# Baverne/VAE-CYCLEGAN-Implementation

Hardware: AMD Instinct MI355X
Metric: train images/sec (256x256 VAE-CycleGAN step) (higher is better)
Workload: dtype f32; 1 GPU; cyclevaegan unpaired, 3x256x256 synthetic summer<->winter, per-GPU batch 8, latent 64 (BASELINE.json configs[3]/[4]); per_gpu_batch=8, global_batch=8, image_size=256, latent_dim=64, parallelism=dp1, init=random (reference init statistics)

## Files before the change

include/vcg.h:

```cpp
#ifndef VCG_H
#define VCG_H

#include <stddef.h>
#include <stdint.h>

#ifdef __cplusplus
extern "C" {
#endif

#define VCG_ABI_VERSION 6

void vcg_amax_hint(uint64_t x_amax, uint64_t dy_amax);
uint64_t vcg_amax_last(void);
uint64_t vcg_amax_measure(const float* t, size_t n, void* stream);
int vcg_amax_valid(uint64_t handle);

enum {
  VCG_CD_N = 0,
  VCG_CD_H = 1,
  VCG_CD_W = 2,
  VCG_CD_CIN = 3,
  VCG_CD_COUT = 4,
  VCG_CD_KH = 5,
  VCG_CD_KW = 6,
  VCG_CD_STRIDE = 7,
  VCG_CD_PAD = 8,
  VCG_CD_REFLECT = 9,
  VCG_CD_UPS = 10,
  VCG_CD_ACT = 11,
  VCG_CD_CIN_LOGICAL = 12,
  VCG_CD_COUT_LOGICAL = 13,
  VCG_CD_PACK_FLAGS = 14,
  VCG_CD_LEN = 16
};

enum { VCG_ACT_NONE = 0, VCG_ACT_RELU = 1, VCG_ACT_LEAKY02 = 2, VCG_ACT_TANH = 3, VCG_ACT_SIGMOID = 4 };

int vcg_abi_version(void);
const char* vcg_last_error(void);

int vcg_profile_enable(int on);
long vcg_profile_read(char* buf, size_t cap);

int vcg_nchw_to_nhwc(const float* src, float* dst, int N, int C, int H, int W, int P, void* stream);
int vcg_nhwc_to_nchw(const float* src, float* dst, int N, int C, int H, int W, int P, void* stream);
int vcg_fill(float* dst, float value, size_t n, void* stream);

size_t vcg_pack_weight_floats(const int32_t* cd);
int vcg_conv_reads_wf(const int32_t* cd);
int vcg_pack_weight(const float* w_oihw, float* wf, const int32_t* cd, void* stream);
size_t vcg_conv_fwd_workspace(const int32_t* cd);
int vcg_conv_fwd(const float* x, const float* wf, const float* bias, float* y,
                 const int32_t* cd, void* ws, size_t ws_bytes, void* stream);

size_t vcg_conv_fwd_in_workspace(const int32_t* cd);
size_t vcg_conv_saved_floats(const int32_t* cd);
int vcg_conv_fwd_in(const float* x, const float* wf, const float* bias, float* y, float* mean, float* rstd, float eps,
                    float* saved, const int32_t* cd, void* ws, size_t ws_bytes, void* stream);
int vcg_conv_fwd_in_h(const float* x, const float* wf, const float* bias, float* y, float* mean, float* rstd, float eps,
                      float* saved, const int32_t* cd, void* ws, size_t ws_bytes, uint64_t x_amax, void* stream);
int vcg_conv_pre_ok(const int32_t* cd);
int vcg_conv_fwd_in_pre(const float* t_prev, const float* pre_mean, const float* pre_rstd, int pre_act, const float* wf,
                        const float* bias, float* y, float* mean, float* rstd, float eps, float* saved, const int32_t* cd,
                        void* ws, size_t ws_bytes, void* stream);
size_t vcg_conv_dgrad_workspace(const int32_t* cd);
int vcg_conv_dgrad(const float* dy, const float* wf, float* dx, const int32_t* cd,
                   void* ws, size_t ws_bytes, void* stream);
int vcg_conv_dgrad_h(const float* dy, const float* wf, float* dx, const int32_t* cd,
                     void* ws, size_t ws_bytes, uint64_t dy_amax, void* stream);
size_t vcg_conv_wgrad_workspace(const int32_t* cd);
int vcg_conv_wgrad(const float* x, const float* dy, float* gw_oihw, float* gbias,
                   const int32_t* cd, void* ws, size_t ws_bytes, void* stream);
int vcg_conv_wgrad_saved(const float* x, const float* dy, float* gw_oihw, float* gbias, const float* saved,
                         const int32_t* cd, void* ws, size_t ws_bytes, void* stream);
int vcg_conv_wgrad_saved_h(const float* x, const float* dy, float* gw_oihw, float* gbias, const float* saved,
                           const int32_t* cd, void* ws, size_t ws_bytes, uint64_t x_amax, uint64_t dy_amax, void* stream);

size_t vcg_in_workspace(int N, int HW, int C);
int vcg_in_stats(const float* t, float* mean, float* rstd, int N, int HW, int C, float eps,
                 void* ws, size_t ws_bytes, void* stream);
int vcg_in_apply(const float* t, const float* mean, const float* rstd, const float* residual,
                 float* out, int N, int H, int W, int C, int post_act, int shuffle, void* stream);
int vcg_in_apply_h(const float* t, const float* mean, const float* rstd, const float* residual,
                   float* out, int N, int H, int W, int C, int post_act, int shuffle, uint64_t* out_amax, void* stream);
int vcg_in_bwd(const float* g, const float* t, const float* mean, const float* rstd, float* dt,
               int N, int H, int W, int C, int epi_act, int post_act, int shuffle,
               void* ws, size_t ws_bytes, void* stream);
int vcg_in_bwd_h(const float* g, const float* t, const float* mean, const float* rstd, float* dt,
                 int N, int H, int W, int C, int epi_act, int post_act, int shuffle,
                 void* ws, size_t ws_bytes, uint64_t* dt_amax, void* stream);
int vcg_in_bwd_bias(const float* g, const float* t, const float* mean, const float* rstd, float* dt,
                    int N, int H, int W, int C, int epi_act, int post_act, int shuffle, float* gbias, int c_log,
                    void* ws, size_t ws_bytes, uint64_t* dt_amax, void* stream);
int vcg_pixel_shuffle(const float* src, float* dst, int N, int H, int W, int C, int inverse, void* stream);
int vcg_act_bwd(const float* g, const float* t, float* dt, size_t n, int act, void* stream);
int vcg_act_bwd_h(const float* g, const float* t, float* dt, size_t n, int act, uint64_t* dt_amax, void* stream);

int vcg_chan_split(const float* src, float* a, float* b, size_t rows, int ca, int cb, void* stream);
int vcg_chan_cat(const float* a, const float* b, float* dst, size_t rows, int ca, int cb, void* stream);
int vcg_add_into(float* dst, float* src, size_t n, void* stream);

int vcg_reparam_fwd(const float* mu, const float* lv, const float* eps, float* eps_out,
                    float* z, float* lvc, size_t n, uint64_t seed, uint64_t offset, void* stream);
int vcg_reparam_bwd(const float* gz, const float* glvc, const float* eps, const float* lv,
                    float* dmu, float* dlv, size_t n, void* stream);
int vcg_randn(float* out, size_t n, uint64_t seed, uint64_t offset, void* stream);
int vcg_rand_uniform(float* out, size_t n, uint64_t seed, uint64_t offset, void* stream);

size_t vcg_reduce_workspace(size_t n);
int vcg_l1_fwd(const float* a, const float* b, float* out, size_t n_phys, size_t n_logical,
               void* ws, size_t ws_bytes, void* stream);
int vcg_l1_bwd(const float* a, const float* b, const float* gout, float* ga, float* gb,
               size_t n_phys, size_t n_logical, void* stream);
int vcg_mse_const_fwd(const float* d, float target, float* out, size_t n, void* stream);
int vcg_mse_const_bwd(const float* d, float target, const float* gout, float* gd, size_t n, void* stream);
enum { VCG_GAN_LSGAN = 0, VCG_GAN_HINGE = 1, VCG_GAN_LOGISTIC = 2 };
int vcg_gan_terms_fwd(const float* real, size_t n_real, const float* fake, size_t n_fake, int objective, double smooth,
                      float* out, void* stream);
int vcg_gan_terms_bwd(const float* real, size_t n_real, const float* fake, size_t n_fake, int objective, double smooth,
                      const float* const* g_out, float* g_real, float* g_fake, void* stream);
int vcg_kl_fwd(const float* mu, const float* lv, float* out, size_t n,
               void* ws, size_t ws_bytes, void* stream);
int vcg_kl_bwd(const float* mu, const float* lv, const float* gout, float* gmu, float* glv,
               size_t n, void* stream);
size_t vcg_kl_fb_workspace(size_t rows, int cp);
int vcg_kl_fb_fwd(const float* mu, const float* lv, float* out3, float* klc, size_t rows, int c, int cp, float floor,
                  void* ws, size_t ws_bytes, void* stream);
int vcg_kl_fb_bwd(const float* mu, const float* lv, const float* gout, const float* klc, float* gmu, float* glv,
                  size_t rows, int c, int cp, float floor, void* stream);
size_t vcg_ssim_loss_workspace(int N, int H, int W);
int vcg_ssim_loss_fwd(const float* a, const float* b, float* out, int N, int H, int W, void* ws, size_t ws_bytes,
                      void* stream);
int vcg_ssim_loss_bwd(const float* a, const float* b, const float* gout, float* ga, int N, int H, int W, void* stream);
size_t vcg_msssim_loss_workspace(int N, int H, int W, int scales);
int vcg_msssim_loss_fwd(const float* a, const float* b, float* out, int N, int H, int W, int scales, void* ws, size_t ws_bytes,
                        void* stream);
int vcg_msssim_loss_bwd(const float* a, const float* b, const float* gout, float* ga, int N, int H, int W, int scales, void* ws,
                        size_t ws_bytes, void* stream);
size_t vcg_grad_loss_workspace(int N, int H, int W, int scales);
int vcg_grad_loss_fwd(const float* a, const float* b, float* out, int N, int H, int W, int scales, void* ws, size_t ws_bytes,
                      void* stream);
int vcg_grad_loss_bwd(const float* a, const float* b, const float* gout, float* ga, int N, int H, int W, int scales,
                      void* stream);
#define VCG_FREQ_MAX_SIDE 2048
size_t vcg_freq_loss_workspace(int N, int H, int W);
size_t vcg_freq_loss_spectrum(int N, int H, int W);
int vcg_freq_loss_fwd(const float* a, const float* b, float* out, int N, int H, int W, float alpha, void* spec,
                      size_t spec_bytes, void* ws, size_t ws_bytes, void* stream);
int vcg_freq_loss_bwd(const void* spec, size_t spec_bytes, const float* gout, float* ga, int N, int H, int W, float alpha,
                      void* ws, size_t ws_bytes, void* stream);
int vcg_lincomb_fwd(const float* const* s, const float* w, int count, float* out, void* stream);

int vcg_sn_prepare(const float* w_orig_oihw, float* u, float* v, float* sigma, float* wsn_k,
                   int C, int KH, int KW, int update_uv, void* ws, size_t ws_bytes, void* stream);
int vcg_fullmap_fwd(const float* x, const float* wsn_k, const float* bias, float* out,
                    int N, size_t K, void* stream);
int vcg_fullmap_dgrad(const float* g, const float* wsn_k, float* dx, int N, size_t K, void* stream);
int vcg_fullmap_wgrad(const float* g, const float* x, const float* wsn_k, const float* sigma,
                      const float* u, const float* v, float* gw_orig_oihw, float* gbias,
                      int N, int C, int KH, int KW, void* ws, size_t ws_bytes, void* stream);

size_t vcg_patch_head_workspace(int N, int H, int W, int C, int KH, int KW);
int vcg_patch_head_fwd(const float* x, const float* wsn_k, const float* bias, float* out, int N, int H, int W, int C, int KH,
                       int KW, void* ws, size_t ws_bytes, void* stream);
int vcg_patch_head_dgrad(const float* g, const float* wsn_k, float* dx, int N, int H, int W, int C, int KH, int KW, void* stream);
int vcg_patch_head_wgrad(const float* g, const float* x, const float* wsn_k, const float* sigma, const float* u, const float* v,
                         float* gw_orig_oihw, float* gbias, int N, int H, int W, int C, int KH, int KW, void* ws, size_t ws_bytes,
                         void* stream);

int vcg_input_resample(const unsigned char* arena, const float* fsrc, const int32_t* params, float* out, int N, int S,
                       void* stream);
int vcg_input_color_jitter(float* img, const float* jitter, int N, int S, void* stream);
int vcg_input_prejitter(const unsigned char* arena, const int32_t* frames, const float* jitter, const int32_t* var,
                        float* fbuf, int N, void* stream);

int vcg_image_metrics(const float* out, const float* target, float* result, int N, int S, float* ws, size_t ws_bytes,
                      void* stream);
int vcg_to_display(const float* x, void* out, int N, int S, int as_uint8, void* stream);

int vcg_image_load(const unsigned char* src, float* out, int N, int H, int W, int C, int Hp, int Wp, int top, int left,
                   void* stream);
int vcg_to_display_hw(const float* x, void* out, int N, int Hp, int Wp, int top, int left, int H, int W, int as_uint8,
                      void* stream);
int vcg_image_metrics_hw(const float* out, const float* target, float* result, int N, int Hp, int Wp, int top, int left,
                         int H, int W, float* ws, size_t ws_bytes, void* stream);

int vcg_adam_step(float* p, const float* g, float* m, float* v, size_t n,
                  float step_size, float beta1, float beta2, float one_minus_beta1, float one_minus_beta2,
                  float eps, float bc2_sqrt, float grad_scale, void* stream);

size_t vcg_grad_norm_workspace(size_t n);
int vcg_grad_norm(const float* g, size_t n, float grad_scale, float max_norm, float* out, void* ws, size_t ws_bytes,
                  void* stream);
int vcg_adam_step_clipped(float* p, const float* g, float* m, float* v, size_t n,
                          float step_size, float beta1, float beta2, float one_minus_beta1, float one_minus_beta2,
                          float eps, float bc2_sqrt, float grad_scale, const float* clip, void* stream);

int vcg_ema_update(float* e, const float* p, size_t n, float w, const float* skip, void* stream);
int vcg_swap(float* a, float* b, size_t n, void* stream);

int vcg_pool_exchange(const float* fake, float* pool, float* out, const int32_t* plan, int N, size_t elems, int capacity,
                      void* stream);

int vcg_reparam_many_fwd(const float* mu, const float* lv, const float* eps, float* eps_out, float* z, int N, int K, int first,
                         int k, size_t per, float temperature, uint64_t seed, uint64_t offset, void* stream);
int vcg_sample_accumulate(const float* y, float* mean, float* m2, int N, int k, int seen, size_t pixels, void* stream);
size_t vcg_spread_workspace(int N, int H, int W);
int vcg_spread_display_hw(const float* m2, int count, float gain, float* out_f32, unsigned char* out_u8, float* result, int N,
                          int Hp, int Wp, int top, int left, int H, int W, void* ws, size_t ws_bytes, void* stream);

#define VCG_SWD_MAX_DESC 16384
int vcg_swd_pyramid_level(const float* g, float* g_next, float* lap, int N, int S, int clamp, void* stream);
int vcg_swd_gather(const float* level, int N, int S, const int32_t* plan, int count, float* out, size_t row_offset,
                   size_t rows, void* stream);
size_t vcg_swd_normalize_workspace(int n);
int vcg_swd_normalize(const float* desc, float* out, int n, void* ws, size_t ws_bytes, void* stream);
int vcg_swd_project(const float* desc, const float* dirs, float* out, int n, int K, int ndir, void* stream);
int vcg_sort_columns(const float* x, float* out, int n, int cols, size_t row_stride, size_t col_stride, void* stream);
size_t vcg_swd_distance_workspace(size_t n);
int vcg_swd_distance(const float* a, const float* b, float* out, size_t n, void* ws, size_t ws_bytes, void* stream);

#define VCG_SWD_LOSS_MAX_DESC 8192
#define VCG_SWD_LOSS_MAX_LEVELS 3
int vcg_swd_loss_levels(int H, int W);
int vcg_swd_cell_side(int N, int H, int W);
int vcg_swd_pool(const float* x, float* out, int N, int H, int W, void* stream);
int vcg_swd_pool_adjoint_add(const float* coarse, float* fine, int N, int H, int W, void* stream);
int vcg_swd_grid_gather(const float* level, float* out, int N, int H, int W, int s, int oy, int ox, void* stream);
int vcg_swd_grid_scatter(const float* gdesc, const float* gscale, float scale, float* out, int N, int H, int W, int s, int oy,
                         int ox, void* stream);
int vcg_sort_columns_indexed(const float* x, float* keys, int32_t* rows, int n, int cols, size_t row_stride, size_t col_stride,
                             void* stream);
size_t vcg_swd_pair_loss_workspace(int n, int ndir);
int vcg_swd_pair_loss(const float* a_sorted, const float* b_sorted, const int32_t* perm_a, float* gproj, int n, int ndir,
                      double weight, int accumulate, double* total, float* out, void* ws, size_t ws_bytes, void* stream);
int vcg_swd_unit_columns(const float* x, float* out, int K, int D, void* stream);

#ifdef __cplusplus
}
#endif
#endif
```

vae-cyclegan-implementation_amd/_native.py:

```python
import ctypes
import os
import subprocess

_HERE = os.path.dirname(os.path.abspath(__file__))
CSRC = os.path.join(_HERE, "csrc")
LIB_PATH = os.environ.get("VCG_LIBVCG") or os.path.join(_HERE, "libvcg.so")
SOURCES = ["conv_igemm.hip", "conv_thin.hip", "conv_thinin.hip", "conv_wino.hip", "conv_slab.hip", "conv_ring.hip", "gemm_split.hip", "norm.hip", "misc.hip", "input.hip", "metrics.hip", "image_io.hip", "ssim_loss.hip", "grad_loss.hip", "freq_loss.hip", "grad_clip.hip", "ema.hip", "image_pool.hip", "sample_stats.hip", "swd.hip", "swd_loss.hip", "msssim_loss.hip", "kl_free_bits.hip", "patch_head.hip", "gan_terms.hip"]
HEADER = os.path.join(os.path.dirname(_HERE), "include", "vcg.h")

_c = ctypes
_P = _c.c_void_p
_I = _c.c_int
_Z = _c.c_size_t
_F = _c.c_float
_D = _c.c_double
_U64 = _c.c_uint64
_I32P = _c.POINTER(_c.c_int32)
_U64P = _c.POINTER(_c.c_uint64)

SIGNATURES = {
    "vcg_abi_version": (_I, []),
    "vcg_last_error": (_c.c_char_p, []),
    "vcg_amax_hint": (None, [_U64, _U64]),
    "vcg_amax_last": (_U64, []),
    "vcg_amax_measure": (_U64, [_P, _Z, _P]),
    "vcg_amax_valid": (_I, [_U64]),
    "vcg_conv_fwd_in_h": (_I, [_P, _P, _P, _P, _P, _P, _F, _P, _I32P, _P, _Z, _U64, _P]),
    "vcg_conv_dgrad_h": (_I, [_P, _P, _P, _I32P, _P, _Z, _U64, _P]),
    "vcg_conv_wgrad_saved_h": (_I, [_P, _P, _P, _P, _P, _I32P, _P, _Z, _U64, _U64, _P]),
    "vcg_in_apply_h": (_I, [_P, _P, _P, _P, _P, _I, _I, _I, _I, _I, _I, _U64P, _P]),
    "vcg_in_bwd_h": (_I, [_P, _P, _P, _P, _P, _I, _I, _I, _I, _I, _I, _I, _P, _Z, _U64P, _P]),
    "vcg_in_bwd_bias": (_I, [_P, _P, _P, _P, _P, _I, _I, _I, _I, _I, _I, _I, _P, _I, _P, _Z, _U64P, _P]),
    "vcg_act_bwd_h": (_I, [_P, _P, _P, _Z, _I, _U64P, _P]),
    "vcg_profile_enable": (_I, [_I]),
    "vcg_profile_read": (_c.c_long, [_c.c_char_p, _Z]),
    "vcg_nchw_to_nhwc": (_I, [_P, _P, _I, _I, _I, _I, _I, _P]),
    "vcg_nhwc_to_nchw": (_I, [_P, _P, _I, _I, _I, _I, _I, _P]),
    "vcg_fill": (_I, [_P, _F, _Z, _P]),
    "vcg_pack_weight_floats": (_Z, [_I32P]),
    "vcg_pack_weight": (_I, [_P, _P, _I32P, _P]),
    "vcg_conv_reads_wf": (_I, [_I32P]),
    "vcg_conv_fwd_workspace": (_Z, [_I32P]),
    "vcg_conv_fwd": (_I, [_P, _P, _P, _P, _I32P, _P, _Z, _P]),
    "vcg_conv_fwd_in_workspace": (_Z, [_I32P]),
    "vcg_conv_saved_floats": (_Z, [_I32P]),
    "vcg_conv_fwd_in": (_I, [_P, _P, _P, _P, _P, _P, _F, _P, _I32P, _P, _Z, _P]),
    "vcg_conv_pre_ok": (_I, [_I32P]),
    "vcg_conv_fwd_in_pre": (_I, [_P, _P, _P, _I, _P, _P, _P, _P, _P, _F, _P, _I32P, _P, _Z, _P]),
    "vcg_conv_wgrad_saved": (_I, [_P, _P, _P, _P, _P, _I32P, _P, _Z, _P]),
    "vcg_conv_dgrad_workspace": (_Z, [_I32P]),
    "vcg_conv_dgrad": (_I, [_P, _P, _P, _I32P, _P, _Z, _P]),
    "vcg_conv_wgrad_workspace": (_Z, [_I32P]),
    "vcg_conv_wgrad": (_I, [_P, _P, _P, _P, _I32P, _P, _Z, _P]),
    "vcg_in_workspace": (_Z, [_I, _I, _I]),
    "vcg_in_stats": (_I, [_P, _P, _P, _I, _I, _I, _F, _P, _Z, _P]),
    "vcg_in_apply": (_I, [_P, _P, _P, _P, _P, _I, _I, _I, _I, _I, _I, _P]),
    "vcg_in_bwd": (_I, [_P, _P, _P, _P, _P, _I, _I, _I, _I, _I, _I, _I, _P, _Z, _P]),
    "vcg_act_bwd": (_I, [_P, _P, _P, _Z, _I, _P]),
    "vcg_pixel_shuffle": (_I, [_P, _P, _I, _I, _I, _I, _I, _P]),
    "vcg_chan_split": (_I, [_P, _P, _P, _Z, _I, _I, _P]),
    "vcg_chan_cat": (_I, [_P, _P, _P, _Z, _I, _I, _P]),
    "vcg_add_into": (_I, [_P, _P, _Z, _P]),
    "vcg_reparam_fwd": (_I, [_P, _P, _P, _P, _P, _P, _Z, _U64, _U64, _P]),
    "vcg_reparam_bwd": (_I, [_P, _P, _P, _P, _P, _P, _Z, _P]),
    "vcg_randn": (_I, [_P, _Z, _U64, _U64, _P]),
    "vcg_rand_uniform": (_I, [_P, _Z, _U64, _U64, _P]),
    "vcg_reduce_workspace": (_Z, [_Z]),
    "vcg_l1_fwd": (_I, [_P, _P, _P, _Z, _Z, _P, _Z, _P]),
    "vcg_l1_bwd": (_I, [_P, _P, _P, _P, _P, _Z, _Z, _P]),
    "vcg_ssim_loss_workspace": (_Z, [_I, _I, _I]),
    "vcg_ssim_loss_fwd": (_I, [_P, _P, _P, _I, _I, _I, _P, _Z, _P]),
    "vcg_ssim_loss_bwd": (_I, [_P, _P, _P, _P, _I, _I, _I, _P]),
    "vcg_msssim_loss_workspace": (_Z, [_I, _I, _I, _I]),
    "vcg_msssim_loss_fwd": (_I, [_P, _P, _P, _I, _I, _I, _I, _P, _Z, _P]),
    "vcg_msssim_loss_bwd": (_I, [_P, _P, _P, _P, _I, _I, _I, _I, _P, _Z, _P]),
    "vcg_grad_loss_workspace": (_Z, [_I, _I, _I, _I]),
    "vcg_grad_loss_fwd": (_I, [_P, _P, _P, _I, _I, _I, _I, _P, _Z, _P]),
    "vcg_grad_loss_bwd": (_I, [_P, _P, _P, _P, _I, _I, _I, _I, _P]),
    "vcg_freq_loss_workspace": (_Z, [_I, _I, _I]),
    "vcg_freq_loss_spectrum": (_Z, [_I, _I, _I]),
    "vcg_freq_loss_fwd": (_I, [_P, _P, _P, _I, _I, _I, _F, _P, _Z, _P, _Z, _P]),
    "vcg_freq_loss_bwd": (_I, [_P, _Z, _P, _P, _I, _I, _I, _F, _P, _Z, _P]),
    "vcg_mse_const_fwd": (_I, [_P, _F, _P, _Z, _P]),
    "vcg_mse_const_bwd": (_I, [_P, _F, _P, _P, _Z, _P]),
    "vcg_gan_terms_fwd": (_I, [_P, _Z, _P, _Z, _I, _D, _P, _P]),
    "vcg_gan_terms_bwd": (_I, [_P, _Z, _P, _Z, _I, _D, _c.POINTER(_P), _P, _P, _P]),
    "vcg_kl_fwd": (_I, [_P, _P, _P, _Z, _P, _Z, _P]),
    "vcg_kl_bwd": (_I, [_P, _P, _P, _P, _P, _Z, _P]),
    "vcg_kl_fb_workspace": (_Z, [_Z, _I]),
    "vcg_kl_fb_fwd": (_I, [_P, _P, _P, _P, _Z, _I, _I, _F, _P, _Z, _P]),
    "vcg_kl_fb_bwd": (_I, [_P, _P, _P, _P, _P, _P, _Z, _I, _I, _F, _P]),
    "vcg_lincomb_fwd": (_I, [_c.POINTER(_P), _c.POINTER(_F), _I, _P, _P]),
    "vcg_sn_prepare": (_I, [_P, _P, _P, _P, _P, _I, _I, _I, _I, _P, _Z, _P]),
    "vcg_fullmap_fwd": (_I, [_P, _P, _P, _P, _I, _Z, _P]),
    "vcg_fullmap_dgrad": (_I, [_P, _P, _P, _I, _Z, _P]),
    "vcg_fullmap_wgrad": (_I, [_P, _P, _P, _P, _P, _P, _P, _P, _I, _I, _I, _I, _P, _Z, _P]),
    "vcg_patch_head_workspace": (_Z, [_I, _I, _I, _I, _I, _I]),
    "vcg_patch_head_fwd": (_I, [_P, _P, _P, _P, _I, _I, _I, _I, _I, _I, _P, _Z, _P]),
    "vcg_patch_head_dgrad": (_I, [_P, _P, _P, _I, _I, _I, _I, _I, _I, _P]),
    "vcg_patch_head_wgrad": (_I, [_P, _P, _P, _P, _P, _P, _P, _P, _I, _I, _I, _I, _I, _I, _P, _Z, _P]),
    "vcg_input_resample": (_I, [_P, _P, _P, _P, _I, _I, _P]),
    "vcg_input_prejitter": (_I, [_P, _P, _P, _P, _P, _I, _P]),
    "vcg_input_color_jitter": (_I, [_P, _P, _I, _I, _P]),
    "vcg_adam_step": (_I, [_P, _P, _P, _P, _Z, _F, _F, _F, _F, _F, _F, _F, _F, _P]),
    "vcg_grad_norm_workspace": (_Z, [_Z]),
    "vcg_grad_norm": (_I, [_P, _Z, _F, _F, _P, _P, _Z, _P]),
    "vcg_adam_step_clipped": (_I, [_P, _P, _P, _P, _Z, _F, _F, _F, _F, _F, _F, _F, _F, _P, _P]),
    "vcg_ema_update": (_I, [_P, _P, _Z, _F, _P, _P]),
    "vcg_swap": (_I, [_P, _P, _Z, _P]),
    "vcg_pool_exchange": (_I, [_P, _P, _P, _I32P, _I, _Z, _I, _P]),
    "vcg_image_metrics": (_I, [_P, _P, _P, _I, _I, _P, _Z, _P]),
    "vcg_to_display": (_I, [_P, _P, _I, _I, _I, _P]),
    "vcg_image_load": (_I, [_P, _P, _I, _I, _I, _I, _I, _I, _I, _I, _P]),
    "vcg_to_display_hw": (_I, [_P, _P, _I, _I, _I, _I, _I, _I, _I, _I, _P]),
    "vcg_image_metrics_hw": (_I, [_P, _P, _P, _I, _I, _I, _I, _I, _I, _I, _P, _Z, _P]),
    "vcg_reparam_many_fwd": (_I, [_P, _P, _P, _P, _P, _I, _I, _I, _I, _Z, _F, _U64, _U64, _P]),
    "vcg_sample_accumulate": (_I, [_P, _P, _P, _I, _I, _I, _Z, _P]),
    "vcg_spread_workspace": (_Z, [_I, _I, _I]),
    "vcg_spread_display_hw": (_I, [_P, _I, _F, _P, _P, _P, _I, _I, _I, _I, _I, _I, _I, _P, _Z, _P]),
    "vcg_swd_pyramid_level": (_I, [_P, _P, _P, _I, _I, _I, _P]),
    "vcg_swd_gather": (_I, [_P, _I, _I, _I32P, _I, _P, _Z, _Z, _P]),
    "vcg_swd_normalize_workspace": (_Z, [_I]),
    "vcg_swd_normalize": (_I, [_P, _P, _I, _P, _Z, _P]),
    "vcg_swd_project": (_I, [_P, _P, _P, _I, _I, _I, _P]),
    "vcg_sort_columns": (_I, [_P, _P, _I, _I, _Z, _Z, _P]),
    "vcg_swd_distance_workspace": (_Z, [_Z]),
    "vcg_swd_distance": (_I, [_P, _P, _P, _Z, _P, _Z, _P]),
    "vcg_swd_loss_levels": (_I, [_I, _I]),
    "vcg_swd_cell_side": (_I, [_I, _I, _I]),
    "vcg_swd_pool": (_I, [_P, _P, _I, _I, _I, _P]),
    "vcg_swd_pool_adjoint_add": (_I, [_P, _P, _I, _I, _I, _P]),
    "vcg_swd_grid_gather": (_I, [_P, _P, _I, _I, _I, _I, _I, _I, _P]),
    "vcg_swd_grid_scatter": (_I, [_P, _P, _F, _P, _I, _I, _I, _I, _I, _I, _P]),
    "vcg_sort_columns_indexed": (_I, [_P, _P, _P, _I, _I, _Z, _Z, _P]),
    "vcg_swd_pair_loss_workspace": (_Z, [_I, _I]),
    "vcg_swd_pair_loss": (_I, [_P, _P, _P, _P, _I, _I, _D, _I, _P, _P, _P, _Z, _P]),
    "vcg_swd_unit_columns": (_I, [_P, _P, _I, _I, _P]),
}

_lib = None
ABI_VERSION = 6


def hipcc_path():
    for cand in (os.environ.get("HIPCC"), "/opt/rocm/bin/hipcc", "hipcc"):
        if cand and (os.path.isabs(cand) and os.path.exists(cand) or not os.path.isabs(cand)):
            return cand
    return "hipcc"


def build(force=False, verbose=False):
    if os.environ.get("VCG_LIBVCG"):
        return LIB_PATH
    srcs = [os.path.join(CSRC, s) for s in SOURCES]
    headers = [os.path.join(CSRC, "vcg_common.h"), os.path.join(CSRC, "ssim_window.h"), HEADER]
    deps = srcs + headers
    if not force and os.path.exists(LIB_PATH):
        if os.path.getmtime(LIB_PATH) >= max(os.path.getmtime(d) for d in deps):
            return LIB_PATH
    from concurrent.futures import ThreadPoolExecutor
    objdir = os.path.join(CSRC, "_obj")
    os.makedirs(objdir, exist_ok=True)
    flags = ["--offload-arch=gfx950", "-O3", "-std=c++17", "-fno-slp-vectorize", "-fPIC"]
    hdr_time = max(os.path.getmtime(h) for h in headers)

    def compile_one(src):
        obj = os.path.join(objdir, os.path.basename(src) + ".o")
        if not force and os.path.exists(obj) and os.path.getmtime(obj) >= max(os.path.getmtime(src), hdr_time):
            return obj, None
        cmd = [hipcc_path()] + flags + ["-c", src, "-o", obj]
        if verbose:
            print(" ".join(cmd), flush=True)
        res = subprocess.run(cmd, capture_output=True, text=True)
        return obj, (res.stdout + res.stderr if res.returncode != 0 else None)

    with ThreadPoolExecutor(max_workers=min(len(srcs), os.cpu_count() or 4)) as pool:
        results = list(pool.map(compile_one, srcs))
    bad = [err for _, err in results if err]
    if bad:
        raise RuntimeError("hipcc failed:\n" + "\n".join(bad))
    tmp = LIB_PATH + f".tmp{os.getpid()}"
    cmd = [hipcc_path(), "--offload-arch=gfx950", "-fPIC", "-shared", "-o", tmp] + [o for o, _ in results]
    if verbose:
        print(" ".join(cmd), flush=True)
    res = subprocess.run(cmd, capture_output=True, text=True)
    if res.returncode != 0:
        raise RuntimeError("hipcc (link) failed:\n" + res.stdout + res.stderr)
    os.replace(tmp, LIB_PATH)
    return LIB_PATH


def lib():
    global _lib
    if _lib is None:
        if not os.path.exists(LIB_PATH):
            raise RuntimeError(
                f"{LIB_PATH} is missing: the HIP extension has not been built "
                "(run `python -c 'import __graft_entry__ as g; g.build()'`). "
                "This package has no fallback path.")
        handle = ctypes.CDLL(LIB_PATH)
        for name, (res, args) in SIGNATURES.items():
            fn = getattr(handle, name)
            fn.restype = res
            fn.argtypes = args
        if handle.vcg_abi_version() != ABI_VERSION:
            raise RuntimeError("libvcg.so ABI version mismatch; rebuild it")
        _lib = handle
    return _lib


def check(rc, what):
    if rc != 0:
        msg = lib().vcg_last_error()
        raise RuntimeError(f"{what} failed (rc={rc}): {msg.decode() if msg else ''}")
```

vae-cyclegan-implementation_amd/csrc/conv_wino.hip:

```cpp
#include "vcg_common.h"
#ifdef VCG_STAMP
#include <stdlib.h>
#endif

#define WINO_U_SHIFT 2
#define WINO_V_SHIFT 2
int vcg_gemm_planes_batched(const void* APlanes, const void* BtPlanes, float* C, int rows, int K, int N, int batches, const VcgAmax& amax_a,
                            const VcgAmax& amax_b, hipStream_t st, uint32_t* amax_a_keep);

struct WinoP {
  const float* x;
  const float* m;
  const float* bias;
  float* y;
  int N, H, W, Cin, Cout, Hl, Wl, ups, reflect, act, cout_log;
  int th, tw, T, Kc;
  int off;
  FastDiv fd_k4, fd_tw, fd_thtw, fd_c4, fd_co4;
  unsigned long long* amax_slot;
  uint32_t amax_gen;
  VcgAmax amax_x;
  unsigned short* vplanes;
  const float* pre_mean;
  const float* pre_rstd;
  int pre_act;
};
__device__ __forceinline__ float4 wino_pre_apply(const float4& v, const float4& mu, const float4& rs, int act) {
  return make_float4(act_apply((v.x - mu.x) * rs.x, act), act_apply((v.y - mu.y) * rs.y, act), act_apply((v.z - mu.z) * rs.z, act),
                     act_apply((v.w - mu.w) * rs.w, act));
}

__device__ __forceinline__ float4 f4sub(const float4& a, const float4& b) { return make_float4(a.x - b.x, a.y - b.y, a.z - b.z, a.w - b.w); }
__device__ __forceinline__ float4 f4sum(const float4& a, const float4& b) { return make_float4(a.x + b.x, a.y + b.y, a.z + b.z, a.w + b.w); }

__global__ __launch_bounds__(256) void k_wino_in_planes(WinoP p) {
  float sc, inv;
  vcg_scale_of(vcg_amax_bits(p.amax_x), p.amax_x.shift, sc, inv);
  const uint32_t k4n = (uint32_t)p.Kc / 4;
  const size_t total = (size_t)p.T * k4n;
  const size_t KB = (size_t)p.Kc / 32;
  for (size_t idx = (size_t)blockIdx.x * blockDim.x + threadIdx.x; idx < total; idx += (size_t)gridDim.x * blockDim.x) {
    const uint32_t t = (uint32_t)(idx / k4n);
    const uint32_t k4 = (uint32_t)(idx - (size_t)t * k4n);
    const uint32_t ph = fd_div(k4, p.fd_c4);
    const int c = (int)(k4 - ph * (uint32_t)(p.Cin / 4)) * 4;
    const int pi = (int)(ph >> 1), pj = (int)(ph & 1);
    const uint32_t n = fd_div(t, p.fd_thtw);
    const uint32_t rem = t - n * (uint32_t)(p.th * p.tw);
    const uint32_t ty = fd_div(rem, p.fd_tw);
    const int tx = (int)(rem - ty * (uint32_t)p.tw);
    const float* xn = p.x + (size_t)n * p.H * p.W * p.Cin;
    float4 pmu = make_float4(0.f, 0.f, 0.f, 0.f), prs = pmu;
    if (p.pre_mean) {
      pmu = *reinterpret_cast<const float4*>(p.pre_mean + (size_t)n * p.Cin + c);
      prs = *reinterpret_cast<const float4*>(p.pre_rstd + (size_t)n * p.Cin + c);
    }
    float4 d[4][4];
#pragma unroll
    for (int r = 0; r < 4; ++r) {
      int ih = 2 * (int)ty - p.off + r;
      bool okh = true;
      if (p.reflect) ih = reflect_idx(ih, p.Hl);
      else okh = ih >= 0 && ih < p.Hl;
#pragma unroll
      for (int s = 0; s < 4; ++s) {
        int iw = 2 * tx - p.off + s;
        bool ok = okh;
        if (p.reflect) iw = reflect_idx(iw, p.Wl);
        else ok = ok && iw >= 0 && iw < p.Wl;
        d[r][s] = ok ? *reinterpret_cast<const float4*>(xn + ((size_t)(ih * p.ups + pi) * p.W + (iw * p.ups + pj)) * p.Cin + c)
                     : make_float4(0.f, 0.f, 0.f, 0.f);
        if (p.pre_mean && ok) d[r][s] = wino_pre_apply(d[r][s], pmu, prs, p.pre_act);
      }
    }
    float4 e[4][4];
#pragma unroll
    for (int s = 0; s < 4; ++s) {
      e[0][s] = f4sub(d[0][s], d[2][s]);
      e[1][s] = f4sum(d[1][s], d[2][s]);
      e[2][s] = f4sub(d[2][s], d[1][s]);
      e[3][s] = f4sub(d[1][s], d[3][s]);
    }
    const uint32_t k = k4 * 4;
    unsigned short* vb = p.vplanes + ((size_t)t * KB + k / 32) * VCG_PBLK + (k & 31);
    const size_t plane = (size_t)p.T * KB * VCG_PBLK;
#pragma unroll
    for (int a = 0; a < 4; ++a) {
      const float4 o[4] = {f4sub(e[a][0], e[a][2]), f4sum(e[a][1], e[a][2]), f4sub(e[a][2], e[a][1]), f4sub(e[a][1], e[a][3])};
#pragma unroll
      for (int b = 0; b < 4; ++b) {
        uint2 h, l;
        split4h(o[b], inv, h, l);
        unsigned short* q = vb + (size_t)(a * 4 + b) * plane;
        *reinterpret_cast<uint2*>(q) = h;
        *reinterpret_cast<uint2*>(q + 32) = l;
      }
    }
  }
}

__global__ __launch_bounds__(256) void k_wino_out(WinoP p) {
  const uint32_t c4n = (uint32_t)p.Cout / 4;
  const size_t total = (size_t)p.T * c4n;
  const size_t plane = (size_t)p.T * p.Cout;
  for (size_t idx = (size_t)blockIdx.x * blockDim.x + threadIdx.x; idx < total; idx += (size_t)gridDim.x * blockDim.x) {
    const uint32_t t = (uint32_t)(idx / c4n);
    const int co = (int)(idx - (size_t)t * c4n) * 4;
    const uint32_t n = fd_div(t, p.fd_thtw);
    const uint32_t rem = t - n * (uint32_t)(p.th * p.tw);
    const uint32_t ty = fd_div(rem, p.fd_tw);
    const int tx = (int)(rem - ty * (uint32_t)p.tw);
    const float* mb = p.m + (size_t)t * p.Cout + co;
    float4 s0[4], s1[4];
#pragma unroll
    for (int b = 0; b < 4; ++b) {
      const float4 m0 = *reinterpret_cast<const float4*>(mb + (size_t)(0 + b) * plane);
      const float4 m1 = *reinterpret_cast<const float4*>(mb + (size_t)(4 + b) * plane);
      const float4 m2 = *reinterpret_cast<const float4*>(mb + (size_t)(8 + b) * plane);
      const float4 m3 = *reinterpret_cast<const float4*>(mb + (size_t)(12 + b) * plane);
      s0[b] = f4sum(f4sum(m0, m1), m2);
      s1[b] = f4sub(f4sub(m1, m2), m3);
    }
    float4 y[2][2];
    y[0][0] = f4sum(f4sum(s0[0], s0[1]), s0[2]);
    y[0][1] = f4sub(f4sub(s0[1], s0[2]), s0[3]);
    y[1][0] = f4sum(f4sum(s1[0], s1[1]), s1[2]);
    y[1][1] = f4sub(f4sub(s1[1], s1[2]), s1[3]);
    float4 bv = make_float4(0.f, 0.f, 0.f, 0.f);
    if (p.bias) {
      if (co + 0 < p.cout_log) bv.x = p.bias[co + 0];
      if (co + 1 < p.cout_log) bv.y = p.bias[co + 1];
      if (co + 2 < p.cout_log) bv.z = p.bias[co + 2];
      if (co + 3 < p.cout_log) bv.w = p.bias[co + 3];
    }
#pragma unroll
    for (int r = 0; r < 2; ++r)
#pragma unroll
      for (int s = 0; s < 2; ++s) {
        const int oh = 2 * (int)ty + r, ow = 2 * tx + s;
        if (oh < p.Hl && ow < p.Wl) {
          float4 o = y[r][s];
          o.x = act_apply(o.x + bv.x, p.act); o.y = act_apply(o.y + bv.y, p.act);
          o.z = act_apply(o.z + bv.z, p.act); o.w = act_apply(o.w + bv.w, p.act);
          *reinterpret_cast<float4*>(p.y + (((size_t)n * p.Hl + oh) * p.Wl + ow) * p.Cout + co) = o;
        }
      }
  }
}

__global__ __launch_bounds__(256) void k_wino_out_stats(WinoP p, double* __restrict__ part, NormPlan pl) {
  __shared__ double r1[256 * 4];
  __shared__ double r2[256 * 4];
  const int tc = threadIdx.x % pl.TC, tp = threadIdx.x / pl.TC;
  const int c4 = blockIdx.z * pl.TC + tc;
  const int n = blockIdx.y;
  const int tiles = p.th * p.tw;
  const int pb = blockIdx.x * pl.chunk;
  int pe = pb + pl.chunk;
  if (pe > tiles) pe = tiles;
  const size_t plane = (size_t)p.T * p.Cout;
  double s1[4] = {0.0, 0.0, 0.0, 0.0}, s2[4] = {0.0, 0.0, 0.0, 0.0};
  if (c4 * 4 < p.Cout) {
    const int co = c4 * 4;
    float4 bv = make_float4(0.f, 0.f, 0.f, 0.f);
    if (p.bias) {
      if (co + 0 < p.cout_log) bv.x = p.bias[co + 0];
      if (co + 1 < p.cout_log) bv.y = p.bias[co + 1];
      if (co + 2 < p.cout_log) bv.z = p.bias[co + 2];
      if (co + 3 < p.cout_log) bv.w = p.bias[co + 3];
    }
    for (int tl = pb + tp; tl < pe; tl += pl.TP) {
      const int ty = tl / p.tw, tx = tl - ty * p.tw;
      const size_t t = (size_t)n * tiles + tl;
      const float* mb = p.m + t * p.Cout + co;
      float4 a0[4], a1[4];
#pragma unroll
      for (int b = 0; b < 4; ++b) {
        const float4 m0 = *reinterpret_cast<const float4*>(mb + (size_t)(0 + b) * plane);
        const float4 m1 = *reinterpret_cast<const float4*>(mb + (size_t)(4 + b) * plane);
        const float4 m2 = *reinterpret_cast<const float4*>(mb + (size_t)(8 + b) * plane);
        const float4 m3 = *reinterpret_cast<const float4*>(mb + (size_t)(12 + b) * plane);
        a0[b] = f4sum(f4sum(m0, m1), m2);
        a1[b] = f4sub(f4sub(m1, m2), m3);
      }
      float4 y[2][2];
      y[0][0] = f4sum(f4sum(a0[0], a0[1]), a0[2]);
      y[0][1] = f4sub(f4sub(a0[1], a0[2]), a0[3]);
      y[1][0] = f4sum(f4sum(a1[0], a1[1]), a1[2]);
      y[1][1] = f4sub(f4sub(a1[1], a1[2]), a1[3]);
#pragma unroll
      for (int r = 0; r < 2; ++r)
#pragma unroll
        for (int q = 0; q < 2; ++q) {
          float4 o = y[r][q];
          o.x = act_apply(o.x + bv.x, p.act); o.y = act_apply(o.y + bv.y, p.act);
          o.z = act_apply(o.z + bv.z, p.act); o.w = act_apply(o.w + bv.w, p.act);
          *reinterpret_cast<float4*>(p.y + (((size_t)n * p.Hl + 2 * ty + r) * p.Wl + 2 * tx + q) * p.Cout + co) = o;
          s1[0] += (double)o.x; s2[0] += (double)o.x * (double)o.x;
          s1[1] += (double)o.y; s2[1] += (double)o.y * (double)o.y;
          s1[2] += (double)o.z; s2[2] += (double)o.z * (double)o.z;
          s1[3] += (double)o.w; s2[3] += (double)o.w * (double)o.w;
        }
    }
  }
#pragma unroll
  for (int e = 0; e < 4; ++e) {
    r1[threadIdx.x * 4 + e] = s1[e];
    r2[threadIdx.x * 4 + e] = s2[e];
  }
  __syncthreads();
  if (tp == 0 && c4 * 4 < p.Cout) {
    for (int k = 1; k < pl.TP; ++k) {
#pragma unroll
      for (int e = 0; e < 4; ++e) {
        s1[e] += r1[(k * pl.TC + tc) * 4 + e];
        s2[e] += r2[(k * pl.TC + tc) * 4 + e];
      }
    }
    double* o = part + (((size_t)n * pl.nchunk + blockIdx.x) * p.Cout + c4 * 4) * 2;
#pragma unroll
    for (int e = 0; e < 4; ++e) {
      o[2 * e] = s1[e];
      o[2 * e + 1] = s2[e];
    }
  }
}

template <bool DGRAD>
__global__ __launch_bounds__(256) void k_wino_weight_planes(const float* __restrict__ w, unsigned short* __restrict__ up, int Cin,
                                                            int Cout, int ups, int cin_log, int cout_log, VcgAmax amax) {
  float sc, inv;
  vcg_scale_of(vcg_amax_bits(amax), amax.shift, sc, inv);
  const int U2 = ups * ups, Kc = U2 * Cin;
  const int NR = DGRAD ? Kc : Cout, KD = DGRAD ? Cout : Kc;
  const size_t total = (size_t)NR * (KD / 4);
  for (size_t idx = (size_t)blockIdx.x * blockDim.x + threadIdx.x; idx < total; idx += (size_t)gridDim.x * blockDim.x) {
    const int n = (int)(idx / (KD / 4)), kk = (int)(idx - (size_t)n * (KD / 4)) * 4;
    float t[16][4];
#pragma unroll
    for (int e = 0; e < 4; ++e) {
      const int co = DGRAD ? kk + e : n, k = DGRAD ? n : kk + e;
      const int ph = k / Cin, c = k - ph * Cin;
      const bool ok = co < cout_log && c < cin_log;
      const float* wp = w + ((size_t)co * (cin_log * U2) + (size_t)c * U2 + ph) * 9;
      float g[3][3];
#pragma unroll
      for (int a = 0; a < 3; ++a)
#pragma unroll
        for (int b = 0; b < 3; ++b) g[a][b] = ok ? (DGRAD ? wp[(2 - a) * 3 + (2 - b)] : wp[a * 3 + b]) : 0.f;
      float h[4][3];
#pragma unroll
      for (int b = 0; b < 3; ++b) {
        h[0][b] = g[0][b];
        h[1][b] = 0.5f * (g[0][b] + g[1][b] + g[2][b]);
        h[2][b] = 0.5f * (g[0][b] - g[1][b] + g[2][b]);
        h[3][b] = g[2][b];
      }
#pragma unroll
      for (int a = 0; a < 4; ++a) {
        t[a * 4 + 0][e] = h[a][0];
        t[a * 4 + 1][e] = 0.5f * (h[a][0] + h[a][1] + h[a][2]);
        t[a * 4 + 2][e] = 0.5f * (h[a][0] - h[a][1] + h[a][2]);
        t[a * 4 + 3][e] = h[a][2];
      }
    }
#pragma unroll
    for (int xi = 0; xi < 16; ++xi) {
      uint2 hh, ll;
      split4h(make_float4(t[xi][0], t[xi][1], t[xi][2], t[xi][3]), inv, hh, ll);
      unsigned short* o = up + (((size_t)xi * NR + n) * (KD / 32) + kk / 32) * VCG_PBLK + (kk & 31);
      *reinterpret_cast<uint2*>(o) = hh;
      *reinterpret_cast<uint2*>(o + 32) = ll;
    }
  }
}

__global__ __launch_bounds__(256) void k_wino_out_pad(const float* __restrict__ m, float* __restrict__ dxp, WinoP p) {
  const uint32_t k4n = (uint32_t)p.Kc / 4;
  const size_t total = (size_t)p.T * k4n;
  const size_t plane = (size_t)p.T * p.Kc;
  const int Hp = 2 * p.th, Wp = 2 * p.tw;
  for (size_t idx = (size_t)blockIdx.x * blockDim.x + threadIdx.x; idx < total; idx += (size_t)gridDim.x * blockDim.x) {
    const uint32_t t = (uint32_t)(idx / k4n);
    const int k = (int)(idx - (size_t)t * k4n) * 4;
    const uint32_t n = fd_div(t, p.fd_thtw);
    const uint32_t rem = t - n * (uint32_t)(p.th * p.tw);
    const uint32_t ty = fd_div(rem, p.fd_tw);
    const int tx = (int)(rem - ty * (uint32_t)p.tw);
    const float* mb = m + (size_t)t * p.Kc + k;
    float4 s0[4], s1[4];
#pragma unroll
    for (int b = 0; b < 4; ++b) {
      const float4 m0 = *reinterpret_cast<const float4*>(mb + (size_t)(0 + b) * plane);
      const float4 m1 = *reinterpret_cast<const float4*>(mb + (size_t)(4 + b) * plane);
      const float4 m2 = *reinterpret_cast<const float4*>(mb + (size_t)(8 + b) * plane);
      const float4 m3 = *reinterpret_cast<const float4*>(mb + (size_t)(12 + b) * plane);
      s0[b] = f4sum(f4sum(m0, m1), m2);
      s1[b] = f4sub(f4sub(m1, m2), m3);
    }
    float* o = dxp + (((size_t)n * Hp + 2 * ty) * Wp + 2 * tx) * p.Kc + k;
    *reinterpret_cast<float4*>(o) = f4sum(f4sum(s0[0], s0[1]), s0[2]);
    *reinterpret_cast<float4*>(o + p.Kc) = f4sub(f4sub(s0[1], s0[2]), s0[3]);
    *reinterpret_cast<float4*>(o + (size_t)Wp * p.Kc) = f4sum(f4sum(s1[0], s1[1]), s1[2]);
    *reinterpret_cast<float4*>(o + (size_t)Wp * p.Kc + p.Kc) = f4sub(f4sub(s1[1], s1[2]), s1[3]);
  }
}

__device__ __forceinline__ float4 wino_out_elem(const float* __restrict__ mb, size_t plane, int rr, int cc) {
  float4 acc = make_float4(0.f, 0.f, 0.f, 0.f);
#pragma unroll
  for (int i = 0; i < 3; ++i) {
    const int xi_r = rr + i;
    const float sr = (rr == 1 && i > 0) ? -1.f : 1.f;
#pragma unroll
    for (int j = 0; j < 3; ++j) {
      const int xi_c = cc + j;
      const float sc = (cc == 1 && j > 0) ? -1.f : 1.f;
      const float4 v = *reinterpret_cast<const float4*>(mb + (size_t)(xi_r * 4 + xi_c) * plane);
      const float sg = sr * sc;
      acc.x += sg * v.x; acc.y += sg * v.y; acc.z += sg * v.z; acc.w += sg * v.w;
    }
  }
  return acc;
}
__global__ __launch_bounds__(256) void k_wino_out_fold(const float* __restrict__ m, float* __restrict__ dx, WinoP p, int Hl, int Wl,
                                                       int Cin, int ups, int reflect) {
  const uint32_t k4n = (uint32_t)p.Kc / 4;
  const size_t total = (size_t)p.T * k4n;
  const size_t plane = (size_t)p.T * p.Kc;
  const int W = Wl * ups;
  for (size_t idx = (size_t)blockIdx.x * blockDim.x + threadIdx.x; idx < total; idx += (size_t)gridDim.x * blockDim.x) {
    const uint32_t t = (uint32_t)(idx / k4n);
    const int k = (int)(idx - (size_t)t * k4n) * 4;
    const uint32_t n = fd_div(t, p.fd_thtw);
    const uint32_t rem = t - n * (uint32_t)(p.th * p.tw);
    const int ty = (int)fd_div(rem, p.fd_tw);
    const int tx = (int)(rem - (uint32_t)ty * (uint32_t)p.tw);
    const float* mb = m + (size_t)t * p.Kc + k;
    float4 s0[4], s1[4];
#pragma unroll
    for (int b = 0; b < 4; ++b) {
      const float4 m0 = *reinterpret_cast<const float4*>(mb + (size_t)(0 + b) * plane);
      const float4 m1 = *reinterpret_cast<const float4*>(mb + (size_t)(4 + b) * plane);
      const float4 m2 = *reinterpret_cast<const float4*>(mb + (size_t)(8 + b) * plane);
      const float4 m3 = *reinterpret_cast<const float4*>(mb + (size_t)(12 + b) * plane);
      s0[b] = f4sum(f4sum(m0, m1), m2);
      s1[b] = f4sub(f4sub(m1, m2), m3);
    }
    float4 o[2][2];
    o[0][0] = f4sum(f4sum(s0[0], s0[1]), s0[2]);
    o[0][1] = f4sub(f4sub(s0[1], s0[2]), s0[3]);
    o[1][0] = f4sum(f4sum(s1[0], s1[1]), s1[2]);
    o[1][1] = f4sub(f4sub(s1[1], s1[2]), s1[3]);
    const int ph = k / Cin, c = k - ph * Cin;
    const int pi = ph >> 1, pj = ph & 1;
#pragma unroll
    for (int r = 0; r < 2; ++r)
#pragma unroll
      for (int q = 0; q < 2; ++q) {
        const int qy = 2 * ty + r, qx = 2 * tx + q;
        if (qy < 1 || qy > Hl || qx < 1 || qx > Wl) continue;
        const int h = qy - 1, w = qx - 1;
        float4 sum = o[r][q];
        if (reflect) {
          int qh[2], qw[2], nh = 1, nw = 1;
          qh[0] = qy; qw[0] = qx;
          if (h == 1) qh[nh++] = 0;
          if (h == Hl - 2) qh[nh++] = Hl + 1;
          if (w == 1) qw[nw++] = 0;
          if (w == Wl - 2) qw[nw++] = Wl + 1;
          for (int a = 0; a < nh; ++a)
            for (int b = 0; b < nw; ++b) {
              if (a == 0 && b == 0) continue;
              const size_t t2 = ((size_t)n * p.th + (qh[a] >> 1)) * p.tw + (qw[b] >> 1);
              const float4 v = wino_out_elem(m + t2 * p.Kc + k, plane, qh[a] & 1, qw[b] & 1);
              sum.x += v.x; sum.y += v.y; sum.z += v.z; sum.w += v.w;
            }
        }
        *reinterpret_cast<float4*>(dx + (((size_t)n * Hl * ups + h * ups + pi) * W + (w * ups + pj)) * Cin + c) = sum;
      }
  }
}
__global__ __launch_bounds__(256) void k_wino_fold(const float* __restrict__ dxp, float* __restrict__ dx, int N, int Hl, int Wl,
                                                   int Cin, int ups, int reflect) {
  const int U2 = ups * ups, Kc = U2 * Cin, c4n = Cin / 4;
  const int Hp = Hl + 2, Wp = Wl + 2, W = Wl * ups;
  const size_t total = (size_t)N * Hl * Wl * U2 * c4n;
  for (size_t idx = (size_t)blockIdx.x * blockDim.x + threadIdx.x; idx < total; idx += (size_t)gridDim.x * blockDim.x) {
    const int c = (int)(idx % c4n) * 4;
    size_t r = idx / c4n;
    const int ph = (int)(r % U2); r /= U2;
    const int w = (int)(r % Wl); r /= Wl;
    const int h = (int)(r % Hl);
    const int n = (int)(r / Hl);
    int qh[2], qw[2], nh = 1, nw = 1;
    qh[0] = h + 1; qw[0] = w + 1;
    if (reflect) {
      if (h == 1) qh[nh++] = 0;
      if (h == Hl - 2) qh[nh++] = Hl + 1;
      if (w == 1) qw[nw++] = 0;
      if (w == Wl - 2) qw[nw++] = Wl + 1;
    }
    float4 s = make_float4(0.f, 0.f, 0.f, 0.f);
    for (int a = 0; a < nh; ++a)
      for (int b = 0; b < nw; ++b) {
        const float4 v = *reinterpret_cast<const float4*>(dxp + (((size_t)n * Hp + qh[a]) * Wp + qw[b]) * Kc + ph * Cin + c);
        s.x += v.x; s.y += v.y; s.z += v.z; s.w += v.w;
      }
    const int pi = ph >> 1, pj = ph & 1;
    *reinterpret_cast<float4*>(dx + (((size_t)n * Hl * ups + h * ups + pi) * W + (w * ups + pj)) * Cin + c) = s;
  }
}

__global__ __launch_bounds__(256) void k_wino_dy(const float* __restrict__ dy, float* __restrict__ dm, WinoP p) {
  __shared__ uint32_t amax_red[4];
  uint32_t amax = 0;
  const uint32_t c4n = (uint32_t)p.Cout / 4;
  const size_t total = (size_t)p.T * c4n;
  const size_t plane = (size_t)p.T * p.Cout;
  for (size_t idx = (size_t)blockIdx.x * blockDim.x + threadIdx.x; idx < total; idx += (size_t)gridDim.x * blockDim.x) {
    const uint32_t t = (uint32_t)(idx / c4n);
    const int co = (int)(idx - (size_t)t * c4n) * 4;
    const uint32_t n = fd_div(t, p.fd_thtw);
    const uint32_t rem = t - n * (uint32_t)(p.th * p.tw);
    const uint32_t ty = fd_div(rem, p.fd_tw);
    const int tx = (int)(rem - ty * (uint32_t)p.tw);
    const float* base = dy + (((size_t)n * p.Hl + 2 * ty) * p.Wl + 2 * tx) * p.Cout + co;
    const float4 y00 = *reinterpret_cast<const float4*>(base);
    const float4 y01 = *reinterpret_cast<const float4*>(base + p.Cout);
    const float4 y10 = *reinterpret_cast<const float4*>(base + (size_t)p.Wl * p.Cout);
    const float4 y11 = *reinterpret_cast<const float4*>(base + (size_t)p.Wl * p.Cout + p.Cout);
    const float4 zero = make_float4(0.f, 0.f, 0.f, 0.f);
    float4 z[4][2];
    z[0][0] = y00;              z[0][1] = y01;
    z[1][0] = f4sum(y00, y10);  z[1][1] = f4sum(y01, y11);
    z[2][0] = f4sub(y00, y10);  z[2][1] = f4sub(y01, y11);
    z[3][0] = f4sub(zero, y10); z[3][1] = f4sub(zero, y11);
    float* mb = dm + (size_t)t * p.Cout + co;
#pragma unroll
    for (int a = 0; a < 4; ++a) {
      const float4 o1 = f4sum(z[a][0], z[a][1]), o2 = f4sub(z[a][0], z[a][1]);
      *reinterpret_cast<float4*>(mb + (size_t)(a * 4 + 0) * plane) = z[a][0];
      *reinterpret_cast<float4*>(mb + (size_t)(a * 4 + 1) * plane) = o1;
      *reinterpret_cast<float4*>(mb + (size_t)(a * 4 + 2) * plane) = o2;
      *reinterpret_cast<float4*>(mb + (size_t)(a * 4 + 3) * plane) = f4sub(zero, z[a][1]);
      amax = max(amax, max(max(vcg_abs_bits4(z[a][0]), vcg_abs_bits4(z[a][1])), max(vcg_abs_bits4(o1), vcg_abs_bits4(o2))));
    }
  }
  if (p.amax_slot) vcg_amax_publish(amax, p.amax_slot, p.amax_gen, amax_red);
}

constexpr int WT_PITCH = 34;
__device__ __forceinline__ void wino_tr_store(unsigned short* __restrict__ sh, const float4* __restrict__ o4, float inv, int tl, int q,
                                              unsigned short* __restrict__ dst, size_t xi_stride, size_t row0, int TB, int tb) {
#pragma unroll
  for (int x = 0; x < 4; ++x) {
    uint2 h, l;
    split4h(o4[x], inv, h, l);
    const unsigned short hv[4] = {(unsigned short)h.x, (unsigned short)(h.x >> 16), (unsigned short)h.y, (unsigned short)(h.y >> 16)};
    const unsigned short lv[4] = {(unsigned short)l.x, (unsigned short)(l.x >> 16), (unsigned short)l.y, (unsigned short)(l.y >> 16)};
#pragma unroll
    for (int e = 0; e < 4; ++e) {
      sh[((x * 2 + 0) * 32 + 4 * q + e) * WT_PITCH + tl] = hv[e];
      sh[((x * 2 + 1) * 32 + 4 * q + e) * WT_PITCH + tl] = lv[e];
    }
  }
  __syncthreads();
  {
    const int pc = threadIdx.x & 1, c = (threadIdx.x >> 1) & 31, x = threadIdx.x >> 6;
    const uint32_t* src = reinterpret_cast<const uint32_t*>(sh + ((x * 2 + pc) * 32 + c) * WT_PITCH);
    uint4 v[4];
#pragma unroll
    for (int j = 0; j < 4; ++j) v[j] = make_uint4(src[4 * j], src[4 * j + 1], src[4 * j + 2], src[4 * j + 3]);
    unsigned short* o = dst + (size_t)x * xi_stride + ((row0 + c) * TB + tb) * VCG_PBLK + pc * 32;
#pragma unroll
    for (int j = 0; j < 4; ++j) *reinterpret_cast<uint4*>(o + 8 * j) = v[j];
  }
  __syncthreads();
}
__global__ __launch_bounds__(256) void k_wino_in_tr(WinoP p, unsigned short* __restrict__ vt) {
  __shared__ __attribute__((aligned(16))) unsigned short sh[4 * 2 * 32 * WT_PITCH];
  float sc, inv;
  vcg_scale_of(vcg_amax_bits(p.amax_x), p.amax_x.shift, sc, inv);
  const int tl = threadIdx.x >> 3, q = threadIdx.x & 7;
  const uint32_t t = blockIdx.x * 32 + tl;
  const uint32_t k4 = blockIdx.y * 8 + q;
  const uint32_t ph = fd_div(k4, p.fd_c4);
  const int c = (int)(k4 - ph * (uint32_t)(p.Cin / 4)) * 4;
  const int pi = (int)(ph >> 1), pj = (int)(ph & 1);
  const uint32_t n = fd_div(t, p.fd_thtw);
  const uint32_t rem = t - n * (uint32_t)(p.th * p.tw);
  const uint32_t ty = fd_div(rem, p.fd_tw);
  const int tx = (int)(rem - ty * (uint32_t)p.tw);
  const float* xn = p.x + (size_t)n * p.H * p.W * p.Cin;
  float4 pmu = make_float4(0.f, 0.f, 0.f, 0.f), prs = pmu;
  if (p.pre_mean) {
    pmu = *reinterpret_cast<const float4*>(p.pre_mean + (size_t)n * p.Cin + c);
    prs = *reinterpret_cast<const float4*>(p.pre_rstd + (size_t)n * p.Cin + c);
  }
  float4 d[4][4];
#pragma unroll
  for (int r = 0; r < 4; ++r) {
    int ih = 2 * (int)ty - p.off + r;
    bool okh = true;
    if (p.reflect) ih = reflect_idx(ih, p.Hl);
    else okh = ih >= 0 && ih < p.Hl;
#pragma unroll
    for (int s = 0; s < 4; ++s) {
      int iw = 2 * tx - p.off + s;
      bool ok = okh;
      if (p.reflect) iw = reflect_idx(iw, p.Wl);
      else ok = ok && iw >= 0 && iw < p.Wl;
      d[r][s] = ok ? *reinterpret_cast<const float4*>(xn + ((size_t)(ih * p.ups + pi) * p.W + (iw * p.ups + pj)) * p.Cin + c)
                   : make_float4(0.f, 0.f, 0.f, 0.f);
      if (p.pre_mean && ok) d[r][s] = wino_pre_apply(d[r][s], pmu, prs, p.pre_act);
    }
  }
  float4 e[4][4];
#pragma unroll
  for (int s = 0; s < 4; ++s) {
    e[0][s] = f4sub(d[0][s], d[2][s]);
    e[1][s] = f4sum(d[1][s], d[2][s]);
    e[2][s] = f4sub(d[2][s], d[1][s]);
    e[3][s] = f4sub(d[1][s], d[3][s]);
  }
  const uint32_t k = k4 * 4;
  const size_t KB = (size_t)p.Kc / 32;
  const int TB = p.T / 32;
#pragma unroll
  for (int a = 0; a < 4; ++a) {
    const float4 o[4] = {f4sub(e[a][0], e[a][2]), f4sum(e[a][1], e[a][2]), f4sub(e[a][2], e[a][1]), f4sub(e[a][1], e[a][3])};
    if (p.vplanes) {
      unsigned short* vb = p.vplanes + ((size_t)t * KB + k / 32) * VCG_PBLK + (k & 31);
      const size_t plane = (size_t)p.T * KB * VCG_PBLK;
#pragma unroll
      for (int b = 0; b < 4; ++b) {
        uint2 h, l;
        split4h(o[b], inv, h, l);
        unsigned short* w = vb + (size_t)(a * 4 + b) * plane;
        *reinterpret_cast<uint2*>(w) = h;
        *reinterpret_cast<uint2*>(w + 32) = l;
      }
    }
    if (vt) wino_tr_store(sh, o, inv, tl, q, vt + (size_t)(a * 4) * p.Kc * TB * VCG_PBLK, (size_t)p.Kc * TB * VCG_PBLK, (size_t)blockIdx.y * 32, TB, (int)blockIdx.x);
  }
}
__global__ __launch_bounds__(256) void k_wino_dy_tr(const float* __restrict__ dy, unsigned short* __restrict__ dmt, WinoP p) {
  __shared__ __attribute__((aligned(16))) unsigned short sh[4 * 2 * 32 * WT_PITCH];
  float sc, inv;
  vcg_scale_of(vcg_amax_bits(p.amax_x), p.amax_x.shift, sc, inv);
  const int tl = threadIdx.x >> 3, q = threadIdx.x & 7;
  const uint32_t t = blockIdx.x * 32 + tl;
  const int co = ((int)blockIdx.y * 8 + q) * 4;
  const uint32_t n = fd_div(t, p.fd_thtw);
  const uint32_t rem = t - n * (uint32_t)(p.th * p.tw);
  const uint32_t ty = fd_div(rem, p.fd_tw);
  const int tx = (int)(rem - ty * (uint32_t)p.tw);
  const float* base = dy + (((size_t)n * p.Hl + 2 * ty) * p.Wl + 2 * tx) * p.Cout + co;
  const float4 y00 = *reinterpret_cast<const float4*>(base);
  const float4 y01 = *reinterpret_cast<const float4*>(base + p.Cout);
  const float4 y10 = *reinterpret_cast<const float4*>(base + (size_t)p.Wl * p.Cout);
  const float4 y11 = *reinterpret_cast<const float4*>(base + (size_t)p.Wl * p.Cout + p.Cout);
  const float4 zero = make_float4(0.f, 0.f, 0.f, 0.f);
  float4 z[4][2];
  z[0][0] = y00;              z[0][1] = y01;
  z[1][0] = f4sum(y00, y10);  z[1][1] = f4sum(y01, y11);
  z[2][0] = f4sub(y00, y10);  z[2][1] = f4sub(y01, y11);
  z[3][0] = f4sub(zero, y10); z[3][1] = f4sub(zero, y11);
  const int TB = p.T / 32;
#pragma unroll
  for (int a = 0; a < 4; ++a) {
    const float4 o[4] = {z[a][0], f4sum(z[a][0], z[a][1]), f4sub(z[a][0], z[a][1]), f4sub(zero, z[a][1])};
    wino_tr_store(sh, o, inv, tl, q, dmt + (size_t)(a * 4) * p.Cout * TB * VCG_PBLK, (size_t)p.Cout * TB * VCG_PBLK, (size_t)blockIdx.y * 32, TB, (int)blockIdx.x);
  }
}

static int wino_blocks(size_t work) {
  size_t b = (work + 255) / 256;
  if (b > 8192) b = 8192;
  return b < 1 ? 1 : (int)b;
}

bool vcg_wino_weight_ok(const ConvGeom& g) {
  return g.KH == 3 && g.KW == 3 && g.stride == 1 && g.pad == 1 && g.ups * g.ups * g.Cin >= 128 && g.Cout >= 64 &&
         g.Cin % 4 == 0 && g.Cout % 64 == 0 && (g.ups * g.ups * g.Cin) % 64 == 0;
}
static bool wino_map_ok(const ConvGeom& g) {
  if (!vcg_wino_weight_ok(g)) return false;
#ifdef VCG_STAMP
  if (getenv("VCG_NO_WINOGRAD")) return false;
#endif
  return !(g.Ho < 4 || g.Wo < 4 || (g.Ho & 1) || (g.Wo & 1));
}
bool vcg_wino_fwd_ok(const ConvGeom& g) {
  if (!wino_map_ok(g)) return false;
  const unsigned long long T = (unsigned long long)g.N * (g.Ho / 2) * (g.Wo / 2);
  const unsigned long long Kc = (unsigned long long)g.ups * g.ups * g.Cin;
  if (Kc * g.Cout < (unsigned long long)kWinoGateFwd * (Kc + g.Cout)) return false;
  return T * Kc * 4 < (1ull << 31) && T * g.Cout * 4 < (1ull << 31) && T * Kc * 16 < (1ull << 32);
}
size_t vcg_wino_weight_floats(const ConvGeom& g) { return (size_t)16 * g.ups * g.ups * g.Cin * g.Cout * VCG_NP / 2; }
size_t vcg_wino_fwd_workspace(const ConvGeom& g) {
  const size_t T = (size_t)g.N * (g.Ho / 2) * (g.Wo / 2);
  return (size_t)16 * T * ((size_t)g.ups * g.ups * g.Cin + g.Cout) * sizeof(float) + 512;
}
int vcg_wino_weight(const ConvGeom& g, const float* w_oihw, float* u, const VcgAmax& amax_w, hipStream_t st) {
  const size_t total = (size_t)g.ups * g.ups * g.Cin * g.Cout / 4;
  VcgAmax au = amax_w; au.shift += WINO_U_SHIFT;
  hipLaunchKernelGGL(k_wino_weight_planes<false>, dim3(wino_blocks(total)), dim3(256), 0, st, w_oihw, (unsigned short*)u, g.Cin, g.Cout,
                     g.ups, g.cin_log, g.cout_log, au);
  VCG_LAUNCH_CHECK("vcg_wino_weight");
  return 0;
}

static WinoP wino_params(const ConvGeom& g) {
  WinoP p = {};
  p.x = nullptr; p.m = nullptr; p.bias = nullptr; p.y = nullptr;
  p.N = g.N; p.H = g.H; p.W = g.W; p.Cin = g.Cin; p.Cout = g.Cout; p.Hl = g.Hl; p.Wl = g.Wl; p.ups = g.ups;
  p.reflect = g.reflect; p.act = g.act; p.cout_log = g.cout_log;
  p.th = g.Ho / 2; p.tw = g.Wo / 2; p.T = g.N * p.th * p.tw; p.Kc = g.ups * g.ups * g.Cin;
  p.fd_k4 = make_fastdiv((uint32_t)p.Kc / 4); p.fd_tw = make_fastdiv((uint32_t)p.tw);
  p.fd_thtw = make_fastdiv((uint32_t)(p.th * p.tw)); p.fd_c4 = make_fastdiv((uint32_t)g.Cin / 4);
  p.fd_co4 = make_fastdiv((uint32_t)g.Cout / 4);
  p.off = 1;
  p.amax_slot = nullptr; p.amax_gen = 0;
  p.amax_x = vcg_amax_const(0); p.vplanes = nullptr;
  p.pre_mean = nullptr; p.pre_rstd = nullptr; p.pre_act = VCG_ACT_NONE;
  return p;
}

bool vcg_wino_wgrad_ok(const ConvGeom& g) {
  const long long kc = (long long)g.ups * g.ups * g.Cin;
  return vcg_wino_fwd_ok(g) && kc % 128 == 0 && kc * g.Cout >= kWinoGateWgrad * (kc + g.Cout);
}
bool vcg_wino_wgrad_tr_ok(const ConvGeom& g) {
  if (!vcg_wino_wgrad_ok(g)) return false;
  const long long kc = (long long)g.ups * g.ups * g.Cin, T = (long long)g.N * (g.Ho / 2) * (g.Wo / 2);
  return T % 32 == 0 && kc % 32 == 0 && g.Cout % 128 == 0 && kc >= 256 && ((kc + 255) / 256) * (g.Cout / 128) * 16 >= 192 &&
         16 * kc * T * VCG_NP < (1ll << 32) && 16 * (long long)g.Cout * T * VCG_NP < (1ll << 32);
}
size_t vcg_wino_wgrad_workspace(const ConvGeom& g) {
  const int T = g.N * (g.Ho / 2) * (g.Wo / 2);
  return vcg_wino_fwd_workspace(g) + vcg_wino_wgrad_core_workspace(g, T);
}
static size_t wino_v_floats(const ConvGeom& g) { return (size_t)16 * g.N * (g.Ho / 2) * (g.Wo / 2) * g.ups * g.ups * g.Cin; }
size_t vcg_wino_saved_floats(const ConvGeom& g) { return vcg_wino_wgrad_ok(g) ? wino_v_floats(g) + 16 : 0; }
int vcg_wino_wgrad(const ConvGeom& g, const float* x, const float* dy, float* gw_oihw, void* ws, size_t ws_bytes, hipStream_t st,
                   const float* v_saved, uint64_t x_handle, uint64_t dy_handle) {
  VCG_CHECK_ARG(ws && ws_bytes >= vcg_wino_wgrad_workspace(g), "vcg_conv_wgrad: workspace too small for the Winograd path");
  WinoP p = wino_params(g);
  float* V = (float*)ws;
  float* dM = V + (((size_t)16 * p.T * p.Kc + 63) / 64) * 64;
  const size_t tbytes = vcg_wino_fwd_workspace(g);
  if (vcg_wino_wgrad_tr_ok(g)) {
    VcgAmax amax_v;
    const unsigned short* Vt;
    if (v_saved) {
      Vt = reinterpret_cast<const unsigned short*>(v_saved);
      amax_v = vcg_amax_stored(v_saved + wino_v_floats(g), WINO_V_SHIFT);
    } else {
      if (vcg_operand_amax(x, (size_t)g.N * g.H * g.W * g.Cin, x_handle, WINO_V_SHIFT, st, &amax_v)) return -2;
      p.x = x; p.amax_x = amax_v; p.vplanes = nullptr;
      hipLaunchKernelGGL(k_wino_in_tr, dim3(p.T / 32, p.Kc / 32), dim3(256), 0, st, p, (unsigned short*)V);
      Vt = reinterpret_cast<const unsigned short*>(V);
    }
    VcgAmax amax_d;
    if (vcg_operand_amax(dy, (size_t)g.N * g.Ho * g.Wo * g.Cout, dy_handle, WINO_V_SHIFT, st, &amax_d)) return -2;
    WinoP pd = p;
    pd.amax_x = amax_d;
    hipLaunchKernelGGL(k_wino_dy_tr, dim3(p.T / 32, g.Cout / 32), dim3(256), 0, st, dy, (unsigned short*)dM, pd);
    VCG_LAUNCH_CHECK("vcg_conv_wgrad(winograd transforms, transposed)");
    float* dU = reinterpret_cast<float*>((char*)ws + tbytes);
    if (vcg_gemm_planes_batched(Vt, dM, dU, p.Kc, p.T, g.Cout, 16, amax_v, amax_d, st, nullptr)) return -2;
    return vcg_wino_wgrad_reduce_one(g, dU, gw_oihw, st);
  }
  p.x = x;
  VcgAmax amax_v;
  if (v_saved) {
    V = const_cast<float*>(v_saved);
    amax_v = vcg_amax_stored(v_saved + wino_v_floats(g), WINO_V_SHIFT);
  } else {
    if (vcg_operand_amax(x, (size_t)g.N * g.H * g.W * g.Cin, x_handle, WINO_V_SHIFT, st, &amax_v)) return -2;
    p.amax_x = amax_v; p.vplanes = (unsigned short*)V;
    hipLaunchKernelGGL(k_wino_in_planes, dim3(wino_blocks((size_t)p.T * p.Kc / 4)), dim3(256), 0, st, p);
  }
  const VcgAmaxOut ad = vcg_amax_new(st);
  p.amax_slot = ad.slot; p.amax_gen = ad.gen;
  hipLaunchKernelGGL(k_wino_dy, dim3(wino_blocks((size_t)p.T * g.Cout / 4)), dim3(256), 0, st, dy, dM, p);
  VCG_LAUNCH_CHECK("vcg_conv_wgrad(winograd transforms)");
  return vcg_wino_wgrad_core(g, V, dM, p.T, gw_oihw, (char*)ws + tbytes, ws_bytes - tbytes, st, amax_v, vcg_amax_in(ad));
}

bool vcg_wino_dgrad_ok(const ConvGeom& g) {
  if (!wino_map_ok(g)) return false;
  const long long kc = (long long)g.ups * g.ups * g.Cin;
  if (kc * g.Cout < kWinoGateDgrad * (kc + g.Cout)) return false;
  const unsigned long long Tp = (unsigned long long)g.N * (g.Ho / 2 + 1) * (g.Wo / 2 + 1);
  return Tp * kc * 4 < (1ull << 31) && Tp * g.Cout * 4 < (1ull << 31) && Tp * g.Cout * 16 < (1ull << 32);
}
size_t vcg_wino_dgrad_workspace(const ConvGeom& g) {
  const size_t Tp = (size_t)g.N * (g.Ho / 2 + 1) * (g.Wo / 2 + 1);
  const size_t kc = (size_t)g.ups * g.ups * g.Cin;
  return (size_t)16 * Tp * (kc + g.Cout) * sizeof(float) + 1024;
}
int vcg_wino_weight_dgrad(const ConvGeom& g, const float* w_oihw, float* ud, const VcgAmax& amax_w, hipStream_t st) {
  const size_t total = (size_t)g.ups * g.ups * g.Cin * g.Cout / 4;
  VcgAmax au = amax_w; au.shift += WINO_U_SHIFT;
  hipLaunchKernelGGL(k_wino_weight_planes<true>, dim3(wino_blocks(total)), dim3(256), 0, st, w_oihw, (unsigned short*)ud, g.Cin, g.Cout,
                     g.ups, g.cin_log, g.cout_log, au);
  VCG_LAUNCH_CHECK("vcg_wino_weight_dgrad");
  return 0;
}
int vcg_wino_dgrad(const ConvGeom& g, const float* dy, const float* ud, const void* w_amax, float* dx, void* ws, size_t ws_bytes,
                   hipStream_t st, uint64_t dy_handle) {
  VCG_CHECK_ARG(ws && ws_bytes >= vcg_wino_dgrad_workspace(g), "vcg_conv_dgrad: workspace too small for the Winograd path");
  const int kc = g.ups * g.ups * g.Cin;
  WinoP p = {};
  p.x = dy; p.bias = nullptr; p.y = nullptr;
  p.N = g.N; p.H = g.Ho; p.W = g.Wo; p.Cin = g.Cout; p.Cout = kc; p.Hl = g.Ho; p.Wl = g.Wo; p.ups = 1;
  p.reflect = 0; p.act = VCG_ACT_NONE; p.cout_log = kc;
  p.th = g.Ho / 2 + 1; p.tw = g.Wo / 2 + 1; p.T = g.N * p.th * p.tw; p.Kc = g.Cout; p.off = 2;
  p.amax_slot = nullptr; p.amax_gen = 0;
  p.amax_x = vcg_amax_const(0); p.vplanes = nullptr;
  p.fd_k4 = make_fastdiv((uint32_t)p.Kc / 4); p.fd_tw = make_fastdiv((uint32_t)p.tw);
  p.fd_thtw = make_fastdiv((uint32_t)(p.th * p.tw)); p.fd_c4 = make_fastdiv((uint32_t)p.Cin / 4);
  p.fd_co4 = make_fastdiv((uint32_t)kc / 4);
  float* V = (float*)ws;
  float* M = V + (((size_t)16 * p.T * g.Cout + 63) / 64) * 64;
  p.m = M;
  VcgAmax ad;
  if (vcg_operand_amax(dy, (size_t)g.N * g.Ho * g.Wo * g.Cout, dy_handle, WINO_V_SHIFT, st, &ad)) return -2;
  p.amax_x = ad; p.vplanes = (unsigned short*)V;
  hipLaunchKernelGGL(k_wino_in_planes, dim3(wino_blocks((size_t)p.T * g.Cout / 4)), dim3(256), 0, st, p);
  VCG_LAUNCH_CHECK("vcg_conv_dgrad(winograd input transform)");
  if (vcg_gemm_planes_batched(V, ud, M, p.T, g.Cout, kc, 16, ad, vcg_amax_stored(w_amax, WINO_U_SHIFT), st, nullptr)) return -2;
  WinoP q = p;
  q.Kc = kc;
  hipLaunchKernelGGL(k_wino_out_fold, dim3(wino_blocks((size_t)p.T * kc / 4)), dim3(256), 0, st, (const float*)M, dx, q, g.Hl, g.Wl,
                     g.Cin, g.ups, g.reflect);
  VCG_LAUNCH_CHECK("vcg_conv_dgrad(winograd output transform)");
  return 0;
}

size_t vcg_wino_fwd_stats_doubles(const ConvGeom& g) {
  const NormPlan pl = vcg_norm_plan(g.N, (g.Ho / 2) * (g.Wo / 2), g.Cout);
  return (size_t)g.N * pl.nchunk * g.Cout * 2;
}
int vcg_wino_fwd(const ConvGeom& g, const float* x, const float* u, const void* w_amax, const float* bias, float* y, void* ws,
                 size_t ws_bytes, hipStream_t st, double* in_part, const VcgInStatsOut* stats, float* v_keep, uint64_t x_handle,
                 const VcgPre* pre) {
  VCG_CHECK_ARG(ws && ws_bytes >= vcg_wino_fwd_workspace(g), "vcg_conv_fwd: workspace too small for the Winograd path (%zu)",
                ws_bytes);
  WinoP p = wino_params(g);
  float* V = v_keep ? v_keep : (float*)ws;
  float* M = (float*)ws + (((size_t)16 * p.T * p.Kc + 63) / 64) * 64;
  p.x = x; p.m = M; p.bias = bias; p.y = y;
  uint32_t pre_bits = 0;
  if (pre && pre->mean) {
    p.pre_mean = pre->mean; p.pre_rstd = pre->rstd; p.pre_act = pre->act;
    const float bound = sqrtf((float)g.H * (float)g.W);
    memcpy(&pre_bits, &bound, 4);
  }
  uint32_t* const keep_word = v_keep ? reinterpret_cast<uint32_t*>(v_keep + wino_v_floats(g)) : nullptr;
  if (v_keep && vcg_wino_wgrad_tr_ok(g)) {
    VcgAmax ax;
    if (pre_bits) ax = vcg_amax_const(pre_bits, WINO_V_SHIFT);
    else if (vcg_operand_amax(x, (size_t)g.N * g.H * g.W * g.Cin, x_handle, WINO_V_SHIFT, st, &ax)) return -2;
    V = (float*)ws;
    p.amax_x = ax; p.vplanes = (unsigned short*)V;
    hipLaunchKernelGGL(k_wino_in_tr, dim3(p.T / 32, p.Kc / 32), dim3(256), 0, st, p, (unsigned short*)v_keep);
    VCG_LAUNCH_CHECK("vcg_conv_fwd(winograd input transform, + transposed)");
    if (vcg_gemm_planes_batched(V, u, M, p.T, p.Kc, g.Cout, 16, ax, vcg_amax_stored(w_amax, WINO_U_SHIFT), st, keep_word)) return -2;
  } else {
    VcgAmax ax;
    if (pre_bits) ax = vcg_amax_const(pre_bits, WINO_V_SHIFT);
    else if (vcg_operand_amax(x, (size_t)g.N * g.H * g.W * g.Cin, x_handle, WINO_V_SHIFT, st, &ax)) return -2;
    p.amax_x = ax; p.vplanes = (unsigned short*)V;
    hipLaunchKernelGGL(k_wino_in_planes, dim3(wino_blocks((size_t)p.T * p.Kc / 4)), dim3(256), 0, st, p);
    VCG_LAUNCH_CHECK("vcg_conv_fwd(winograd input transform)");
    if (vcg_gemm_planes_batched(V, u, M, p.T, p.Kc, g.Cout, 16, ax, vcg_amax_stored(w_amax, WINO_U_SHIFT), st, keep_word)) return -2;
  }
  if (in_part) {
    const NormPlan pl = vcg_norm_plan(g.N, p.th * p.tw, g.Cout);
    hipLaunchKernelGGL(k_wino_out_stats, dim3(pl.nchunk, g.N, pl.cgroups), dim3(256), 0, st, p, in_part, pl);
    VCG_LAUNCH_CHECK("vcg_conv_fwd(winograd output transform)");
    return vcg_in_finalize(in_part, stats->mean, stats->rstd, g.N, stats->HW, g.Cout, pl.nchunk, stats->eps, st);
  } else {
    hipLaunchKernelGGL(k_wino_out, dim3(wino_blocks((size_t)p.T * g.Cout / 4)), dim3(256), 0, st, p);
  }
  VCG_LAUNCH_CHECK("vcg_conv_fwd(winograd output transform)");
  return 0;
}
```

vae-cyclegan-implementation_amd/csrc/gemm_split.hip:

```cpp
#include "vcg_common.h"

typedef unsigned int u32x4g __attribute__((ext_vector_type(4)));

struct GemmSplitP {
  const float* a;
  const float* bt;
  float* c;
  int rows, K, N;
  uint32_t a_bytes, b_bytes;
  uint32_t a_bstride, b_bstride;
  size_t c_bstride;
  VcgAmax amax_a, amax_b;
  uint32_t* amax_a_keep;
};

#define GS_OOB 0x80000000u

template <int BN>
__global__ __launch_bounds__(256, 2) void k_gemm_split(GemmSplitP p) {
  constexpr int BM = 128, NI = BN / 64, MI = 2;
  __shared__ __attribute__((aligned(16))) unsigned char As[VCG_NP][BM * 64];
  __shared__ __attribute__((aligned(16))) unsigned char Bs[VCG_NP][BN * 64];
  const int tid = threadIdx.x, lane = tid & 63, wid = tid >> 6;
  const int wm = wid >> 1, wn = wid & 1, l31 = lane & 31, lh = lane >> 5;
  float sa_, inv_a, sb_, inv_b;
  {
    const uint32_t abits = vcg_amax_bits(p.amax_a);
    vcg_scale_of(abits, p.amax_a.shift, sa_, inv_a);
    vcg_scale_of(vcg_amax_bits(p.amax_b), p.amax_b.shift, sb_, inv_b);
    if (p.amax_a_keep && tid == 0 && blockIdx.x == 0 && blockIdx.y == 0 && blockIdx.z == 0) *p.amax_a_keep = abits;
  }
  int mt, nt, zb;
  {
    const uint32_t per = gridDim.x * gridDim.y, nwg = per * gridDim.z;
    const uint32_t gid = blockIdx.x + gridDim.x * (blockIdx.y + gridDim.y * blockIdx.z);
    const uint32_t q = nwg >> 3, r = nwg & 7, xcd = gid & 7;
    const uint32_t swz = (xcd < r ? xcd * (q + 1) : r * (q + 1) + (xcd - r) * q) + (gid >> 3);
    zb = (int)(swz / per);
    const uint32_t l = swz - (uint32_t)zb * per;
    mt = (int)(l / gridDim.y);
    nt = (int)(l - (uint32_t)mt * gridDim.y);
  }
  const int m0 = mt * BM, n0 = nt * BN;
  const __amdgpu_buffer_rsrc_t ra = __builtin_amdgcn_make_buffer_rsrc((void*)((const unsigned short*)p.a + (size_t)zb * p.a_bstride), 0, (int)p.a_bytes, 0x00020000),
                               rb = __builtin_amdgcn_make_buffer_rsrc((void*)((const unsigned short*)p.bt + (size_t)zb * p.b_bstride), 0, (int)p.b_bytes, 0x00020000);
  constexpr int BP = VCG_NP * BN / 64;
  const int b_q = tid & 3, b_r = tid >> 2;
  const int KB = p.K / 32;
  const uint32_t boff0 = (uint32_t)(((size_t)(n0 + b_r) * KB) * VCG_PBYTES + b_q * 16);
  const uint32_t bhalf = (uint32_t)KB * (64u * VCG_PBYTES);
  const uint32_t bsoff0 = (uint32_t)(b_r * 64 + ((b_q ^ ((b_r >> 2) & 3)) << 4));

  f32x16 acc[MI][NI], lo[MI][NI];
#pragma unroll
  for (int i = 0; i < MI; ++i)
#pragma unroll
    for (int j = 0; j < NI; ++j)
#pragma unroll
      for (int e = 0; e < 16; ++e) acc[i][j][e] = lo[i][j][e] = 0.f;

  u32x4g vb[BP], vap[2 * VCG_NP];
  uint32_t apoff[2];
#pragma unroll
  for (int h = 0; h < 2; ++h) {
    const int r = m0 + b_r + 64 * h;
    apoff[h] = r < p.rows ? (uint32_t)(((size_t)r * KB) * VCG_PBYTES + b_q * 16) : GS_OOB;
  }
  const int nkt = KB;
  auto load_tiles = [&](int kt) {
#pragma unroll
    for (int j = 0; j < 2 * VCG_NP; ++j)
      vap[j] = __builtin_amdgcn_raw_buffer_load_b128(
          ra, (int)(apoff[j / VCG_NP] != GS_OOB ? apoff[j / VCG_NP] + (uint32_t)(j % VCG_NP) * 64u + (uint32_t)kt * VCG_PBYTES : GS_OOB), 0, 0);
#pragma unroll
    for (int j = 0; j < BP; ++j)
      vb[j] = __builtin_amdgcn_raw_buffer_load_b128(rb, (int)(boff0 + (uint32_t)(j / VCG_NP) * bhalf + (uint32_t)(j % VCG_NP) * 64u + (uint32_t)kt * VCG_PBYTES), 0, 0);
  };
  auto store_tiles = [&]() {
#pragma unroll
    for (int j = 0; j < 2 * VCG_NP; ++j) *reinterpret_cast<u32x4g*>(&As[j % VCG_NP][bsoff0 + 4096 * (j / VCG_NP)]) = vap[j];
#pragma unroll
    for (int j = 0; j < BP; ++j) *reinterpret_cast<u32x4g*>(&Bs[j % VCG_NP][bsoff0 + 4096 * (j / VCG_NP)]) = vb[j];
  };
  uint32_t fa[MI], fb[NI];
  int sa[MI], sb[NI];
#pragma unroll
  for (int i = 0; i < MI; ++i) { const int r = wm * 64 + i * 32 + l31; fa[i] = (uint32_t)(r * 64); sa[i] = (r >> 2) & 3; }
#pragma unroll
  for (int j = 0; j < NI; ++j) { const int r = wn * (BN / 2) + j * 32 + l31; fb[j] = (uint32_t)(r * 64); sb[j] = (r >> 2) & 3; }

  load_tiles(0);
  store_tiles();
  __syncthreads();
  for (int kt = 0; kt < nkt; ++kt) {
    if (kt + 1 < nkt) load_tiles(kt + 1);
#pragma unroll
    for (int s = 0; s < 2; ++s) {
      f16x8 a[VCG_NP][MI], b[VCG_NP][NI];
#pragma unroll
      for (int pc = 0; pc < VCG_NP; ++pc) {
#pragma unroll
        for (int i = 0; i < MI; ++i)
          a[pc][i] = *reinterpret_cast<const f16x8*>(&As[pc][fa[i] + (((2 * s + lh) ^ sa[i]) << 4)]);
#pragma unroll
        for (int j = 0; j < NI; ++j)
          b[pc][j] = *reinterpret_cast<const f16x8*>(&Bs[pc][fb[j] + (((2 * s + lh) ^ sb[j]) << 4)]);
      }
#pragma unroll
      for (int i = 0; i < MI; ++i)
#pragma unroll
        for (int j = 0; j < NI; ++j) {
          f32x16 c = lo[i][j];
          c = VCG_MFMA(a[1][i], b[0][j], c);
          c = VCG_MFMA(a[0][i], b[1][j], c);
          lo[i][j] = c;
          acc[i][j] = VCG_MFMA(a[0][i], b[0][j], acc[i][j]);
        }
    }
    __syncthreads();
    if (kt + 1 < nkt) {
      store_tiles();
      __syncthreads();
    }
  }
  float* const dst = p.c + (size_t)zb * p.c_bstride;
  const float os = sa_ * sb_;
#pragma unroll
  for (int j = 0; j < NI; ++j) {
    const int n = n0 + wn * (BN / 2) + j * 32 + l31;
    if (n >= p.N) continue;
#pragma unroll
    for (int i = 0; i < MI; ++i)
#pragma unroll
      for (int e = 0; e < 16; ++e) {
        const int row = (e & 3) + 8 * (e >> 2) + 4 * lh;
        const int m = m0 + wm * 64 + i * 32 + row;
        if (m < p.rows) dst[(size_t)m * p.N + n] = (acc[i][j][e] + lo[i][j][e]) * os;
      }
  }
}

struct GdSrd { uint32_t x, y, z, w; };
typedef uint32_t gd_u32x4 __attribute__((ext_vector_type(4)));
__device__ __forceinline__ gd_u32x4 gd_srd(const void* ptr, uint32_t bytes) {
  const uint64_t a = (uint64_t)ptr;
  gd_u32x4 r;
  r.x = __builtin_amdgcn_readfirstlane((uint32_t)a);
  r.y = __builtin_amdgcn_readfirstlane((uint32_t)(a >> 32) & 0xFFFFu);
  r.z = __builtin_amdgcn_readfirstlane(bytes);
  r.w = 0x00020000u;
  return r;
}
__device__ __forceinline__ void gd_dma16(gd_u32x4 srd, uint32_t lds_dst, uint32_t voff) {
  uint32_t keep;
  asm volatile("s_mov_b32 %0, m0\n\ts_mov_b32 m0, %2\n\ts_nop 0\n\tbuffer_load_dwordx4 %1, %3, 0 offen lds\n\ts_mov_b32 m0, %0"
               : "=&s"(keep) : "v"(voff), "s"(lds_dst), "s"(srd) : "memory");
}
__device__ __forceinline__ void gd_barrier() {
  asm volatile("s_waitcnt lgkmcnt(0)\n\ts_barrier" ::: "memory");
}
constexpr int GD_BM = 256, GD_BN = 128;
constexpr int GD_A_BYTES = GD_BM * VCG_PBYTES, GD_B_BYTES = GD_BN * VCG_PBYTES;
constexpr int GD_STAGE = GD_A_BYTES + GD_B_BYTES;
constexpr int GD_STAGES = 3;
#ifdef VCG_GD_STAMP
__device__ unsigned long long* g_gd_stamp = nullptr;
int vcg_gd_set_stamp(void* buf) { return hipMemcpyToSymbol(HIP_SYMBOL(g_gd_stamp), &buf, sizeof(buf)) == hipSuccess ? 0 : -1; }
#define GD_T() (__builtin_amdgcn_sched_barrier(0), __builtin_amdgcn_s_memtime())
#define GD_ACC(slot, t0) do { const unsigned long long t1__ = GD_T(); gd_acc[slot] += t1__ - (t0); (t0) = t1__; } while (0)
#else
#define GD_T() 0ull
#define GD_ACC(slot, t0) do { } while (0)
#endif
__global__ __launch_bounds__(512, 1) void k_gemm_planes_dma(GemmSplitP p) {
  __shared__ __attribute__((aligned(1024))) unsigned char smem[GD_STAGES * GD_STAGE];
  const int tid = threadIdx.x, lane = tid & 63, wid = tid >> 6;
  const int wm = wid >> 1, wn = wid & 1;
  float sa_, inv_a, sb_, inv_b;
  {
    const uint32_t abits = vcg_amax_bits(p.amax_a);
    vcg_scale_of(abits, p.amax_a.shift, sa_, inv_a);
    vcg_scale_of(vcg_amax_bits(p.amax_b), p.amax_b.shift, sb_, inv_b);
    if (p.amax_a_keep && tid == 0 && blockIdx.x == 0 && blockIdx.y == 0 && blockIdx.z == 0) *p.amax_a_keep = abits;
  }
  int mt, nt, zb;
  {
    const uint32_t per = gridDim.x * gridDim.y, nwg = per * gridDim.z;
    const uint32_t gid = blockIdx.x + gridDim.x * (blockIdx.y + gridDim.y * blockIdx.z);
    const uint32_t q = nwg >> 3, r = nwg & 7, xcd = gid & 7;
    const uint32_t swz = (xcd < r ? xcd * (q + 1) : r * (q + 1) + (xcd - r) * q) + (gid >> 3);
    zb = (int)(swz / per);
    const uint32_t l = swz - (uint32_t)zb * per;
    mt = (int)(l / gridDim.y);
    nt = (int)(l - (uint32_t)mt * gridDim.y);
  }
  const int m0 = mt * GD_BM, n0 = nt * GD_BN;
  const gd_u32x4 ra = gd_srd((const unsigned short*)p.a + (size_t)zb * p.a_bstride, p.a_bytes),
                 rb = gd_srd((const unsigned short*)p.bt + (size_t)zb * p.b_bstride, p.b_bytes);
  const int KB = p.K / 32;
  const int drow = lane >> 3, dslot = lane & 7;
  uint32_t aoff[4], boff[2];
#pragma unroll
  for (int h = 0; h < 4; ++h) {
    const int rl = (wid + 8 * h) * 8 + drow;
    const int r = m0 + rl;
    aoff[h] = r < p.rows ? (uint32_t)((size_t)r * KB * VCG_PBYTES + ((dslot ^ ((rl >> 1) & 7)) << 4)) : GS_OOB;
  }
#pragma unroll
  for (int h = 0; h < 2; ++h) {
    const int rl = (wid + 8 * h) * 8 + drow;
    boff[h] = (uint32_t)((size_t)(n0 + rl) * KB * VCG_PBYTES + ((dslot ^ ((rl >> 1) & 7)) << 4));
  }
  const uint32_t lds0 = (uint32_t)(uintptr_t)(__attribute__((address_space(3))) unsigned char*)smem;
  auto issue_one = [&](int stage, int kt, int q) {
    const uint32_t sbase = __builtin_amdgcn_readfirstlane(lds0 + (uint32_t)stage * GD_STAGE);
    const uint32_t ko = (uint32_t)kt * VCG_PBYTES;
    if (q < 4) gd_dma16(ra, __builtin_amdgcn_readfirstlane(sbase + (uint32_t)((wid + 8 * q) * 1024)), aoff[q] != GS_OOB ? aoff[q] + ko : GS_OOB);
    else gd_dma16(rb, __builtin_amdgcn_readfirstlane(sbase + (uint32_t)(GD_A_BYTES + (wid + 8 * (q - 4)) * 1024)), boff[q - 4] + ko);
  };
  auto issue = [&](int stage, int kt) {
#pragma unroll
    for (int q = 0; q < 6; ++q) issue_one(stage, kt, q);
  };

  f32x4 acc16[4][4], lo16[4][4];
#pragma unroll
  for (int i = 0; i < 4; ++i)
#pragma unroll
    for (int j = 0; j < 4; ++j)
#pragma unroll
      for (int e = 0; e < 4; ++e) acc16[i][j][e] = lo16[i][j][e] = 0.f;
  const int r16 = lane & 15, kq = lane >> 4;
  uint32_t fa16[4], fb16[4];
  int sa16[4], sb16[4];
#pragma unroll
  for (int i = 0; i < 4; ++i) { const int r = wm * 64 + i * 16 + r16; fa16[i] = (uint32_t)(r * VCG_PBYTES); sa16[i] = (r >> 1) & 7; }
#pragma unroll
  for (int j = 0; j < 4; ++j) { const int r = wn * 64 + j * 16 + r16; fb16[j] = (uint32_t)(GD_A_BYTES + r * VCG_PBYTES); sb16[j] = (r >> 1) & 7; }

  const int nkt = KB;
#ifdef VCG_GD_STAMP
  unsigned long long gd_acc[8] = {0, 0, 0, 0, 0, 0, 0, 0};
  const unsigned long long gd_start = GD_T(), gd_rt0 = __builtin_amdgcn_s_memrealtime();
#endif
  issue(0, 0);
  if (nkt > 1) issue(1, 1);
  unsigned long long gd_t = GD_T();
  (void)gd_t;
  f16x8 a16[VCG_NP][4], b16[VCG_NP][4];
  auto read16 = [&](int kt) {
    const unsigned char* st = smem + (kt % GD_STAGES) * GD_STAGE;
#pragma unroll
    for (int pc = 0; pc < VCG_NP; ++pc) {
#pragma unroll
      for (int i = 0; i < 4; ++i)
        a16[pc][i] = *reinterpret_cast<const f16x8*>(st + fa16[i] + (((pc * 4 + kq) ^ sa16[i]) << 4));
#pragma unroll
      for (int j = 0; j < 4; ++j)
        b16[pc][j] = *reinterpret_cast<const f16x8*>(st + fb16[j] + (((pc * 4 + kq) ^ sb16[j]) << 4));
    }
  };
  auto mma16 = [&](int dkt) {
    const bool more = dkt < nkt;
    const int nstage = dkt % GD_STAGES;
    int q = 0;
#pragma unroll
    for (int i = 0; i < 4; ++i)
#pragma unroll
      for (int j = 0; j < 4; ++j) {
        f32x4 c = lo16[i][j];
        c = __builtin_amdgcn_mfma_f32_16x16x32_f16(a16[1][i], b16[0][j], c, 0, 0, 0);
        c = __builtin_amdgcn_mfma_f32_16x16x32_f16(a16[0][i], b16[1][j], c, 0, 0, 0);
        lo16[i][j] = c;
        acc16[i][j] = __builtin_amdgcn_mfma_f32_16x16x32_f16(a16[0][i], b16[0][j], acc16[i][j], 0, 0, 0);
        if ((j & 1) && q < 6) {
          __builtin_amdgcn_sched_barrier(0);
          if (more) issue_one(nstage, dkt, q);
          __builtin_amdgcn_sched_barrier(0);
          ++q;
        }
      }
  };
  const bool late = wid >= 4;
  for (int kt = 0; kt < nkt; ++kt) {
    if (kt + 1 < nkt) asm volatile("s_waitcnt vmcnt(6)" ::: "memory");
    else asm volatile("s_waitcnt vmcnt(0)" ::: "memory");
    GD_ACC(0, gd_t);
    gd_barrier();
    GD_ACC(1, gd_t);
    if (!late) {
      read16(kt);
      mma16(kt + 2);
    } else {
      if (kt > 0) mma16(kt + 2);
      else if (kt + 2 < nkt) issue((kt + 2) % GD_STAGES, kt + 2);
      __builtin_amdgcn_sched_barrier(0);
      read16(kt);
    }
    GD_ACC(2, gd_t);
  }
  if (late) {
    asm volatile("s_waitcnt lgkmcnt(0)" ::: "memory");
    mma16(nkt);
  }
  float* const dst = p.c + (size_t)zb * p.c_bstride;
  const float os = sa_ * sb_;
#pragma unroll
  for (int j = 0; j < 4; ++j) {
    const int n = n0 + wn * 64 + j * 16 + r16;
    if (n >= p.N) continue;
#pragma unroll
    for (int i = 0; i < 4; ++i)
#pragma unroll
      for (int e = 0; e < 4; ++e) {
        const int m = m0 + wm * 64 + i * 16 + 4 * kq + e;
        if (m < p.rows) dst[(size_t)m * p.N + n] = (acc16[i][j][e] + lo16[i][j][e]) * os;
      }
  }
#ifdef VCG_GD_STAMP
  GD_ACC(3, gd_t);
  if (g_gd_stamp && lane == 0) {
    unsigned long long* o = g_gd_stamp + ((size_t)(blockIdx.x + gridDim.x * (blockIdx.y + gridDim.y * blockIdx.z)) * 8 + wid) * 8;
    o[0] = gd_acc[0]; o[1] = gd_acc[1]; o[2] = gd_acc[2]; o[3] = gd_acc[3];
    o[6] = __builtin_amdgcn_s_memrealtime() - gd_rt0; o[7] = gd_t - gd_start;
  }
#endif
}
__global__ __launch_bounds__(256) void k_split_planes(const float* __restrict__ x, unsigned short* __restrict__ bp, size_t quads, int K, VcgAmax amax) {
  float s, inv;
  vcg_scale_of(vcg_amax_bits(amax), amax.shift, s, inv);
  for (size_t i = (size_t)blockIdx.x * blockDim.x + threadIdx.x; i < quads; i += (size_t)gridDim.x * blockDim.x) {
    const size_t e = i * 4, row = e / K;
    const int k = (int)(e - row * K);
    uint2 h, l;
    split4h(*reinterpret_cast<const float4*>(x + e), inv, h, l);
    unsigned short* o = bp + (row * (K / 32) + k / 32) * VCG_PBLK + (k & 31);
    *reinterpret_cast<uint2*>(o) = h;
    *reinterpret_cast<uint2*>(o + 32) = l;
  }
}
int vcg_split_planes(const float* x, void* bp, size_t rows, int K, const VcgAmax& amax, hipStream_t st) {
  VCG_CHECK_ARG(K % 32 == 0, "vcg_split_planes: K must be a multiple of 32");
  const size_t quads = rows * K / 4;
  size_t blocks = (quads + 255) / 256; if (blocks > 8192) blocks = 8192;
  hipLaunchKernelGGL(k_split_planes, dim3((unsigned)blocks), dim3(256), 0, st, x, (unsigned short*)bp, quads, K, amax);
  VCG_LAUNCH_CHECK("vcg_split_planes");
  return 0;
}

int vcg_gemm_planes_batched(const void* APlanes, const void* BtPlanes, float* C, int rows, int K, int N, int batches, const VcgAmax& amax_a,
                            const VcgAmax& amax_b, hipStream_t st, uint32_t* amax_a_keep) {
  VCG_CHECK_ARG(K % 32 == 0 && N % 64 == 0 && rows > 0, "vcg_gemm_planes_batched: bad shape rows=%d K=%d N=%d", rows, K, N);
  VCG_CHECK_ARG((unsigned long long)rows * K * 2 * VCG_NP < (1ull << 31) && (unsigned long long)N * K * 2 * VCG_NP < (1ull << 31),
                "vcg_gemm_planes_batched: operand extents must stay below 2 GiB per batch");
  VCG_CHECK_ARG((unsigned long long)rows * K * VCG_NP * (unsigned long long)batches < (1ull << 32) &&
                    (unsigned long long)N * K * VCG_NP * (unsigned long long)batches < (1ull << 32),
                "vcg_gemm_planes_batched: batch stride overflow");
  GemmSplitP p;
  p.a = (const float*)APlanes; p.bt = (const float*)BtPlanes; p.c = C; p.rows = rows; p.K = K; p.N = N;
  p.a_bytes = (uint32_t)((size_t)rows * K * 2 * VCG_NP); p.b_bytes = (uint32_t)((size_t)N * K * 2 * VCG_NP);
  p.a_bstride = (uint32_t)((size_t)rows * K * VCG_NP); p.b_bstride = (uint32_t)((size_t)N * K * VCG_NP);
  p.c_bstride = (size_t)rows * N;
  p.amax_a = amax_a; p.amax_b = amax_b; p.amax_a_keep = amax_a_keep;
  const int bn = (N % 128 == 0) ? 128 : 64;
  if (bn == 128 && rows >= 256) {
    dim3 grid((rows + GD_BM - 1) / GD_BM, N / GD_BN, batches);
    VcgProfScope prof("k_gemm_planes_dma", 2.0 * rows * (double)K * N * batches, st);
    hipLaunchKernelGGL(k_gemm_planes_dma, grid, dim3(512), 0, st, p);
    VCG_LAUNCH_CHECK("vcg_gemm_planes_batched(dma)");
    return 0;
  }
  dim3 grid((rows + 127) / 128, N / bn, batches);
  VcgProfScope prof(bn == 128 ? "k_gemm_split<128, planes>" : "k_gemm_split<64, planes>", 2.0 * rows * (double)K * N * batches, st);
  if (bn == 128) hipLaunchKernelGGL((k_gemm_split<128>), grid, dim3(256), 0, st, p);
  else hipLaunchKernelGGL((k_gemm_split<64>), grid, dim3(256), 0, st, p);
  VCG_LAUNCH_CHECK("vcg_gemm_planes_batched");
  return 0;
}
```

Measured before the change: 247.5 images/s.

## Use tile-major Winograd wgrad with LDS transpose reads instead of transposed operand copies

Replaces the shared-memory transposing Winograd input and dy transform kernels with plain tile-major plane writers. It adds a TN variant of the DMA plane GEMM that reads K-major operands using ds_read_tr16 transposing LDS loads. The forward pass no longer writes a second transposed copy of V, and the wgrad GEMM consumes the same tile-major layout directly. This removes transpose staging, saves memory traffic, and adds new exported entry points, at the cost of a new swizzle and addressing scheme in the GEMM.

```diff
diff --git a/include/vcg.h b/include/vcg.h
--- a/include/vcg.h
+++ b/include/vcg.h
@@ -75,6 +75,13 @@
                          const int32_t* cd, void* ws, size_t ws_bytes, void* stream);
 int vcg_conv_wgrad_saved_h(const float* x, const float* dy, float* gw_oihw, float* gbias, const float* saved,
                            const int32_t* cd, void* ws, size_t ws_bytes, uint64_t x_amax, uint64_t dy_amax, void* stream);
+int vcg_conv_wgrad_route(const int32_t* cd);
+size_t vcg_wino_v_floats(const int32_t* cd);
+size_t vcg_wino_wgrad_tn_workspace(const int32_t* cd);
+int vcg_wino_v_planes(const float* x, const float* pre_mean, const float* pre_rstd, int pre_act, float* v, const int32_t* cd,
+                      void* stream);
+int vcg_wino_wgrad_tn(const float* x, const float* dy, float* gw_oihw, const float* v, const int32_t* cd, void* ws,
+                      size_t ws_bytes, void* stream);
 
 size_t vcg_in_workspace(int N, int HW, int C);
 int vcg_in_stats(const float* t, float* mean, float* rstd, int N, int HW, int C, float eps,
diff --git a/vae-cyclegan-implementation_amd/_native.py b/vae-cyclegan-implementation_amd/_native.py
--- a/vae-cyclegan-implementation_amd/_native.py
+++ b/vae-cyclegan-implementation_amd/_native.py
@@ -48,6 +48,11 @@
     "vcg_conv_pre_ok": (_I, [_I32P]),
     "vcg_conv_fwd_in_pre": (_I, [_P, _P, _P, _I, _P, _P, _P, _P, _P, _F, _P, _I32P, _P, _Z, _P]),
     "vcg_conv_wgrad_saved": (_I, [_P, _P, _P, _P, _P, _I32P, _P, _Z, _P]),
+    "vcg_conv_wgrad_route": (_I, [_I32P]),
+    "vcg_wino_v_floats": (_Z, [_I32P]),
+    "vcg_wino_wgrad_tn_workspace": (_Z, [_I32P]),
+    "vcg_wino_v_planes": (_I, [_P, _P, _P, _I, _P, _I32P, _P]),
+    "vcg_wino_wgrad_tn": (_I, [_P, _P, _P, _P, _I32P, _P, _Z, _P]),
     "vcg_conv_dgrad_workspace": (_Z, [_I32P]),
     "vcg_conv_dgrad": (_I, [_P, _P, _P, _I32P, _P, _Z, _P]),
     "vcg_conv_wgrad_workspace": (_Z, [_I32P]),
diff --git a/vae-cyclegan-implementation_amd/csrc/conv_wino.hip b/vae-cyclegan-implementation_amd/csrc/conv_wino.hip
--- a/vae-cyclegan-implementation_amd/csrc/conv_wino.hip
+++ b/vae-cyclegan-implementation_amd/csrc/conv_wino.hip
@@ -7,6 +7,8 @@
 #define WINO_V_SHIFT 2
 int vcg_gemm_planes_batched(const void* APlanes, const void* BtPlanes, float* C, int rows, int K, int N, int batches, const VcgAmax& amax_a,
                             const VcgAmax& amax_b, hipStream_t st, uint32_t* amax_a_keep);
+int vcg_gemm_planes_tn_batched(const void* APlanes, const void* BPlanes, float* C, int rows, int T, int N, int batches, const VcgAmax& amax_a,
+                               const VcgAmax& amax_b, hipStream_t st);
 
 struct WinoP {
   const float* x;
@@ -450,128 +452,44 @@
   if (p.amax_slot) vcg_amax_publish(amax, p.amax_slot, p.amax_gen, amax_red);
 }
 
-constexpr int WT_PITCH = 34;
-__device__ __forceinline__ void wino_tr_store(unsigned short* __restrict__ sh, const float4* __restrict__ o4, float inv, int tl, int q,
-                                              unsigned short* __restrict__ dst, size_t xi_stride, size_t row0, int TB, int tb) {
-#pragma unroll
-  for (int x = 0; x < 4; ++x) {
-    uint2 h, l;
-    split4h(o4[x], inv, h, l);
-    const unsigned short hv[4] = {(unsigned short)h.x, (unsigned short)(h.x >> 16), (unsigned short)h.y, (unsigned short)(h.y >> 16)};
-    const unsigned short lv[4] = {(unsigned short)l.x, (unsigned short)(l.x >> 16), (unsigned short)l.y, (unsigned short)(l.y >> 16)};
-#pragma unroll
-    for (int e = 0; e < 4; ++e) {
-      sh[((x * 2 + 0) * 32 + 4 * q + e) * WT_PITCH + tl] = hv[e];
-      sh[((x * 2 + 1) * 32 + 4 * q + e) * WT_PITCH + tl] = lv[e];
-    }
-  }
-  __syncthreads();
-  {
-    const int pc = threadIdx.x & 1, c = (threadIdx.x >> 1) & 31, x = threadIdx.x >> 6;
-    const uint32_t* src = reinterpret_cast<const uint32_t*>(sh + ((x * 2 + pc) * 32 + c) * WT_PITCH);
-    uint4 v[4];
-#pragma unroll
-    for (int j = 0; j < 4; ++j) v[j] = make_uint4(src[4 * j], src[4 * j + 1], src[4 * j + 2], src[4 * j + 3]);
-    unsigned short* o = dst + (size_t)x * xi_stride + ((row0 + c) * TB + tb) * VCG_PBLK + pc * 32;
-#pragma unroll
-    for (int j = 0; j < 4; ++j) *reinterpret_cast<uint4*>(o + 8 * j) = v[j];
-  }
-  __syncthreads();
-}
-__global__ __launch_bounds__(256) void k_wino_in_tr(WinoP p, unsigned short* __restrict__ vt) {
-  __shared__ __attribute__((aligned(16))) unsigned short sh[4 * 2 * 32 * WT_PITCH];
+__global__ __launch_bounds__(256) void k_wino_dy_planes(const float* __restrict__ dy, unsigned short* __restrict__ dmp, WinoP p) {
   float sc, inv;
   vcg_scale_of(vcg_amax_bits(p.amax_x), p.amax_x.shift, sc, inv);
-  const int tl = threadIdx.x >> 3, q = threadIdx.x & 7;
-  const uint32_t t = blockIdx.x * 32 + tl;
-  const uint32_t k4 = blockIdx.y * 8 + q;
-  const uint32_t ph = fd_div(k4, p.fd_c4);
-  const int c = (int)(k4 - ph * (uint32_t)(p.Cin / 4)) * 4;
-  const int pi = (int)(ph >> 1), pj = (int)(ph & 1);
-  const uint32_t n = fd_div(t, p.fd_thtw);
-  const uint32_t rem = t - n * (uint32_t)(p.th * p.tw);
-  const uint32_t ty = fd_div(rem, p.fd_tw);
-  const int tx = (int)(rem - ty * (uint32_t)p.tw);
-  const float* xn = p.x + (size_t)n * p.H * p.W * p.Cin;
-  float4 pmu = make_float4(0.f, 0.f, 0.f, 0.f), prs = pmu;
-  if (p.pre_mean) {
-    pmu = *reinterpret_cast<const float4*>(p.pre_mean + (size_t)n * p.Cin + c);
-    prs = *reinterpret_cast<const float4*>(p.pre_rstd + (size_t)n * p.Cin + c);
-  }
-  float4 d[4][4];
-#pragma unroll
-  for (int r = 0; r < 4; ++r) {
-    int ih = 2 * (int)ty - p.off + r;
-    bool okh = true;
-    if (p.reflect) ih = reflect_idx(ih, p.Hl);
-    else okh = ih >= 0 && ih < p.Hl;
-#pragma unroll
-    for (int s = 0; s < 4; ++s) {
-      int iw = 2 * tx - p.off + s;
-      bool ok = okh;
-      if (p.reflect) iw = reflect_idx(iw, p.Wl);
-      else ok = ok && iw >= 0 && iw < p.Wl;
-      d[r][s] = ok ? *reinterpret_cast<const float4*>(xn + ((size_t)(ih * p.ups + pi) * p.W + (iw * p.ups + pj)) * p.Cin + c)
-                   : make_float4(0.f, 0.f, 0.f, 0.f);
-      if (p.pre_mean && ok) d[r][s] = wino_pre_apply(d[r][s], pmu, prs, p.pre_act);
-    }
-  }
-  float4 e[4][4];
-#pragma unroll
-  for (int s = 0; s < 4; ++s) {
-    e[0][s] = f4sub(d[0][s], d[2][s]);
-    e[1][s] = f4sum(d[1][s], d[2][s]);
-    e[2][s] = f4sub(d[2][s], d[1][s]);
-    e[3][s] = f4sub(d[1][s], d[3][s]);
-  }
-  const uint32_t k = k4 * 4;
-  const size_t KB = (size_t)p.Kc / 32;
-  const int TB = p.T / 32;
-#pragma unroll
-  for (int a = 0; a < 4; ++a) {
-    const float4 o[4] = {f4sub(e[a][0], e[a][2]), f4sum(e[a][1], e[a][2]), f4sub(e[a][2], e[a][1]), f4sub(e[a][1], e[a][3])};
-    if (p.vplanes) {
-      unsigned short* vb = p.vplanes + ((size_t)t * KB + k / 32) * VCG_PBLK + (k & 31);
-      const size_t plane = (size_t)p.T * KB * VCG_PBLK;
+  const uint32_t c4n = (uint32_t)p.Cout / 4;
+  const size_t total = (size_t)p.T * c4n;
+  const size_t CB = (size_t)p.Cout / 32;
+  const size_t plane = (size_t)p.T * CB * VCG_PBLK;
+  for (size_t idx = (size_t)blockIdx.x * blockDim.x + threadIdx.x; idx < total; idx += (size_t)gridDim.x * blockDim.x) {
+    const uint32_t t = (uint32_t)(idx / c4n);
+    const int co = (int)(idx - (size_t)t * c4n) * 4;
+    const uint32_t n = fd_div(t, p.fd_thtw);
+    const uint32_t rem = t - n * (uint32_t)(p.th * p.tw);
+    const uint32_t ty = fd_div(rem, p.fd_tw);
+    const int tx = (int)(rem - ty * (uint32_t)p.tw);
+    const float* base = dy + (((size_t)n * p.Hl + 2 * ty) * p.Wl + 2 * tx) * p.Cout + co;
+    const float4 y00 = *reinterpret_cast<const float4*>(base);
+    const float4 y01 = *reinterpret_cast<const float4*>(base + p.Cout);
+    const float4 y10 = *reinterpret_cast<const float4*>(base + (size_t)p.Wl * p.Cout);
+    const float4 y11 = *reinterpret_cast<const float4*>(base + (size_t)p.Wl * p.Cout + p.Cout);
+    const float4 zero = make_float4(0.f, 0.f, 0.f, 0.f);
+    float4 z[4][2];
+    z[0][0] = y00;              z[0][1] = y01;
+    z[1][0] = f4sum(y00, y10);  z[1][1] = f4sum(y01, y11);
+    z[2][0] = f4sub(y00, y10);  z[2][1] = f4sub(y01, y11);
+    z[3][0] = f4sub(zero, y10); z[3][1] = f4sub(zero, y11);
+    unsigned short* mb = dmp + ((size_t)t * CB + co / 32) * VCG_PBLK + (co & 31);
+#pragma unroll
+    for (int a = 0; a < 4; ++a) {
+      const float4 o[4] = {z[a][0], f4sum(z[a][0], z[a][1]), f4sub(z[a][0], z[a][1]), f4sub(zero, z[a][1])};
 #pragma unroll
       for (int b = 0; b < 4; ++b) {
         uint2 h, l;
         split4h(o[b], inv, h, l);
-        unsigned short* w = vb + (size_t)(a * 4 + b) * plane;
-        *reinterpret_cast<uint2*>(w) = h;
-        *reinterpret_cast<uint2*>(w + 32) = l;
-      }
-    }
-    if (vt) wino_tr_store(sh, o, inv, tl, q, vt + (size_t)(a * 4) * p.Kc * TB * VCG_PBLK, (size_t)p.Kc * TB * VCG_PBLK, (size_t)blockIdx.y * 32, TB, (int)blockIdx.x);
-  }
-}
-__global__ __launch_bounds__(256) void k_wino_dy_tr(const float* __restrict__ dy, unsigned short* __restrict__ dmt, WinoP p) {
-  __shared__ __attribute__((aligned(16))) unsigned short sh[4 * 2 * 32 * WT_PITCH];
-  float sc, inv;
-  vcg_scale_of(vcg_amax_bits(p.amax_x), p.amax_x.shift, sc, inv);
-  const int tl = threadIdx.x >> 3, q = threadIdx.x & 7;
-  const uint32_t t = blockIdx.x * 32 + tl;
-  const int co = ((int)blockIdx.y * 8 + q) * 4;
-  const uint32_t n = fd_div(t, p.fd_thtw);
-  const uint32_t rem = t - n * (uint32_t)(p.th * p.tw);
-  const uint32_t ty = fd_div(rem, p.fd_tw);
-  const int tx = (int)(rem - ty * (uint32_t)p.tw);
-  const float* base = dy + (((size_t)n * p.Hl + 2 * ty) * p.Wl + 2 * tx) * p.Cout + co;
-  const float4 y00 = *reinterpret_cast<const float4*>(base);
-  const float4 y01 = *reinterpret_cast<const float4*>(base + p.Cout);
-  const float4 y10 = *reinterpret_cast<const float4*>(base + (size_t)p.Wl * p.Cout);
-  const float4 y11 = *reinterpret_cast<const float4*>(base + (size_t)p.Wl * p.Cout + p.Cout);
-  const float4 zero = make_float4(0.f, 0.f, 0.f, 0.f);
-  float4 z[4][2];
-  z[0][0] = y00;              z[0][1] = y01;
-  z[1][0] = f4sum(y00, y10);  z[1][1] = f4sum(y01, y11);
-  z[2][0] = f4sub(y00, y10);  z[2][1] = f4sub(y01, y11);
-  z[3][0] = f4sub(zero, y10); z[3][1] = f4sub(zero, y11);
-  const int TB = p.T / 32;
-#pragma unroll
-  for (int a = 0; a < 4; ++a) {
-    const float4 o[4] = {z[a][0], f4sum(z[a][0], z[a][1]), f4sub(z[a][0], z[a][1]), f4sub(zero, z[a][1])};
-    wino_tr_store(sh, o, inv, tl, q, dmt + (size_t)(a * 4) * p.Cout * TB * VCG_PBLK, (size_t)p.Cout * TB * VCG_PBLK, (size_t)blockIdx.y * 32, TB, (int)blockIdx.x);
+        unsigned short* q = mb + (size_t)(a * 4 + b) * plane;
+        *reinterpret_cast<uint2*>(q) = h;
+        *reinterpret_cast<uint2*>(q + 32) = l;
+      }
+    }
   }
 }
 
@@ -645,6 +563,30 @@
 }
 static size_t wino_v_floats(const ConvGeom& g) { return (size_t)16 * g.N * (g.Ho / 2) * (g.Wo / 2) * g.ups * g.ups * g.Cin; }
 size_t vcg_wino_saved_floats(const ConvGeom& g) { return vcg_wino_wgrad_ok(g) ? wino_v_floats(g) + 16 : 0; }
+static int wino_wgrad_tn(const ConvGeom& g, const float* x, const float* dy, float* gw_oihw, void* ws, hipStream_t st,
+                         const float* v_saved, uint64_t x_handle, uint64_t dy_handle) {
+  WinoP p = wino_params(g);
+  float* V = (float*)ws;
+  float* dM = V + (((size_t)16 * p.T * p.Kc + 63) / 64) * 64;
+  VcgAmax amax_v;
+  if (v_saved) {
+    V = const_cast<float*>(v_saved);
+    amax_v = vcg_amax_stored(v_saved + wino_v_floats(g), WINO_V_SHIFT);
+  } else {
+    if (vcg_operand_amax(x, (size_t)g.N * g.H * g.W * g.Cin, x_handle, WINO_V_SHIFT, st, &amax_v)) return -2;
+    p.x = x; p.amax_x = amax_v; p.vplanes = (unsigned short*)V;
+    hipLaunchKernelGGL(k_wino_in_planes, dim3(wino_blocks((size_t)p.T * p.Kc / 4)), dim3(256), 0, st, p);
+  }
+  VcgAmax amax_d;
+  if (vcg_operand_amax(dy, (size_t)g.N * g.Ho * g.Wo * g.Cout, dy_handle, WINO_V_SHIFT, st, &amax_d)) return -2;
+  WinoP pd = p;
+  pd.amax_x = amax_d;
+  hipLaunchKernelGGL(k_wino_dy_planes, dim3(wino_blocks((size_t)p.T * g.Cout / 4)), dim3(256), 0, st, dy, (unsigned short*)dM, pd);
+  VCG_LAUNCH_CHECK("vcg_conv_wgrad(winograd transforms, tile-major)");
+  float* dU = reinterpret_cast<float*>((char*)ws + vcg_wino_fwd_workspace(g));
+  if (vcg_gemm_planes_tn_batched(V, dM, dU, p.Kc, p.T, g.Cout, 16, amax_v, amax_d, st)) return -2;
+  return vcg_wino_wgrad_reduce_one(g, dU, gw_oihw, st);
+}
 int vcg_wino_wgrad(const ConvGeom& g, const float* x, const float* dy, float* gw_oihw, void* ws, size_t ws_bytes, hipStream_t st,
                    const float* v_saved, uint64_t x_handle, uint64_t dy_handle) {
   VCG_CHECK_ARG(ws && ws_bytes >= vcg_wino_wgrad_workspace(g), "vcg_conv_wgrad: workspace too small for the Winograd path");
@@ -652,28 +594,7 @@
   float* V = (float*)ws;
   float* dM = V + (((size_t)16 * p.T * p.Kc + 63) / 64) * 64;
   const size_t tbytes = vcg_wino_fwd_workspace(g);
-  if (vcg_wino_wgrad_tr_ok(g)) {
-    VcgAmax amax_v;
-    const unsigned short* Vt;
-    if (v_saved) {
-      Vt = reinterpret_cast<const unsigned short*>(v_saved);
-      amax_v = vcg_amax_stored(v_saved + wino_v_floats(g), WINO_V_SHIFT);
-    } else {
-      if (vcg_operand_amax(x, (size_t)g.N * g.H * g.W * g.Cin, x_handle, WINO_V_SHIFT, st, &amax_v)) return -2;
-      p.x = x; p.amax_x = amax_v; p.vplanes = nullptr;
-      hipLaunchKernelGGL(k_wino_in_tr, dim3(p.T / 32, p.Kc / 32), dim3(256), 0, st, p, (unsigned short*)V);
-      Vt = reinterpret_cast<const unsigned short*>(V);
-    }
-    VcgAmax amax_d;
-    if (vcg_operand_amax(dy, (size_t)g.N * g.Ho * g.Wo * g.Cout, dy_handle, WINO_V_SHIFT, st, &amax_d)) return -2;
-    WinoP pd = p;
-    pd.amax_x = amax_d;
-    hipLaunchKernelGGL(k_wino_dy_tr, dim3(p.T / 32, g.Cout / 32), dim3(256), 0, st, dy, (unsigned short*)dM, pd);
-    VCG_LAUNCH_CHECK("vcg_conv_wgrad(winograd transforms, transposed)");
-    float* dU = reinterpret_cast<float*>((char*)ws + tbytes);
-    if (vcg_gemm_planes_batched(Vt, dM, dU, p.Kc, p.T, g.Cout, 16, amax_v, amax_d, st, nullptr)) return -2;
-    return vcg_wino_wgrad_reduce_one(g, dU, gw_oihw, st);
-  }
+  if (vcg_wino_wgrad_tr_ok(g)) return wino_wgrad_tn(g, x, dy, gw_oihw, ws, st, v_saved, x_handle, dy_handle);
   p.x = x;
   VcgAmax amax_v;
   if (v_saved) {
@@ -689,6 +610,62 @@
   hipLaunchKernelGGL(k_wino_dy, dim3(wino_blocks((size_t)p.T * g.Cout / 4)), dim3(256), 0, st, dy, dM, p);
   VCG_LAUNCH_CHECK("vcg_conv_wgrad(winograd transforms)");
   return vcg_wino_wgrad_core(g, V, dM, p.T, gw_oihw, (char*)ws + tbytes, ws_bytes - tbytes, st, amax_v, vcg_amax_in(ad));
+}
+
+static bool wino_wgrad_tn_can(const ConvGeom& g) {
+  if (!wino_map_ok(g)) return false;
+  const unsigned long long T = (unsigned long long)g.N * (g.Ho / 2) * (g.Wo / 2), kc = (unsigned long long)g.ups * g.ups * g.Cin;
+  return T % 32 == 0 && kc % 32 == 0 && T * kc * 4 < (1ull << 31) && T * g.Cout * 4 < (1ull << 31) && 16 * kc * T * VCG_NP < (1ull << 32) &&
+         16 * (unsigned long long)g.Cout * T * VCG_NP < (1ull << 32);
+}
+extern "C" int vcg_conv_wgrad_route(const int32_t* cd) {
+  ConvGeom g;
+  if (vcg_conv_geom(cd, &g, "vcg_conv_wgrad_route")) return -1;
+  return !vcg_wino_wgrad_ok(g) ? 0 : vcg_wino_wgrad_tr_ok(g) ? 2 : 1;
+}
+extern "C" size_t vcg_wino_v_floats(const int32_t* cd) {
+  ConvGeom g;
+  if (vcg_conv_geom(cd, &g, "vcg_wino_v_floats")) return 0;
+  return wino_wgrad_tn_can(g) ? wino_v_floats(g) + 16 : 0;
+}
+extern "C" size_t vcg_wino_wgrad_tn_workspace(const int32_t* cd) {
+  ConvGeom g;
+  if (vcg_conv_geom(cd, &g, "vcg_wino_wgrad_tn_workspace")) return 0;
+  return wino_wgrad_tn_can(g) ? vcg_wino_fwd_workspace(g) + (size_t)16 * g.ups * g.ups * g.Cin * g.Cout * sizeof(float) + 256 : 0;
+}
+__global__ __launch_bounds__(64) void k_wino_keep_word(VcgAmax a, uint32_t* __restrict__ dst) {
+  const uint32_t bits = vcg_amax_bits(a);
+  if (threadIdx.x == 0) *dst = bits;
+}
+extern "C" int vcg_wino_v_planes(const float* x, const float* pre_mean, const float* pre_rstd, int pre_act, float* v, const int32_t* cd,
+                                 void* stream) {
+  ConvGeom g;
+  if (vcg_conv_geom(cd, &g, "vcg_wino_v_planes")) return -1;
+  VCG_CHECK_ARG(x && v && wino_wgrad_tn_can(g), "vcg_wino_v_planes: null pointer, or a geometry the tile-major weight gradient cannot run");
+  hipStream_t st = (hipStream_t)stream;
+  WinoP p = wino_params(g);
+  VcgAmax ax;
+  if (pre_mean) {
+    const float bound = sqrtf((float)g.H * (float)g.W);
+    uint32_t bits;
+    memcpy(&bits, &bound, 4);
+    ax = vcg_amax_const(bits, WINO_V_SHIFT);
+    p.pre_mean = pre_mean; p.pre_rstd = pre_rstd; p.pre_act = pre_act;
+  } else if (vcg_operand_amax(x, (size_t)g.N * g.H * g.W * g.Cin, 0, WINO_V_SHIFT, st, &ax)) return -2;
+  p.x = x; p.amax_x = ax; p.vplanes = (unsigned short*)v;
+  hipLaunchKernelGGL(k_wino_in_planes, dim3(wino_blocks((size_t)p.T * p.Kc / 4)), dim3(256), 0, st, p);
+  hipLaunchKernelGGL(k_wino_keep_word, dim3(1), dim3(64), 0, st, ax, reinterpret_cast<uint32_t*>(v + wino_v_floats(g)));
+  VCG_LAUNCH_CHECK("vcg_wino_v_planes");
+  return 0;
+}
+extern "C" int vcg_wino_wgrad_tn(const float* x, const float* dy, float* gw_oihw, const float* v, const int32_t* cd, void* ws,
+                                 size_t ws_bytes, void* stream) {
+  ConvGeom g;
+  if (vcg_conv_geom(cd, &g, "vcg_wino_wgrad_tn")) return -1;
+  VCG_CHECK_ARG((x || v) && dy && gw_oihw && ws, "vcg_wino_wgrad_tn: null pointer");
+  VCG_CHECK_ARG(wino_wgrad_tn_can(g), "vcg_wino_wgrad_tn: a geometry the tile-major weight gradient cannot run (T %% 32, 3x3 stride 1)");
+  VCG_CHECK_ARG(ws_bytes >= vcg_wino_wgrad_tn_workspace(cd), "vcg_wino_wgrad_tn: workspace too small");
+  return wino_wgrad_tn(g, x, dy, gw_oihw, ws, (hipStream_t)stream, v, 0, 0);
 }
 
 bool vcg_wino_dgrad_ok(const ConvGeom& g) {
@@ -762,16 +739,7 @@
     memcpy(&pre_bits, &bound, 4);
   }
   uint32_t* const keep_word = v_keep ? reinterpret_cast<uint32_t*>(v_keep + wino_v_floats(g)) : nullptr;
-  if (v_keep && vcg_wino_wgrad_tr_ok(g)) {
-    VcgAmax ax;
-    if (pre_bits) ax = vcg_amax_const(pre_bits, WINO_V_SHIFT);
-    else if (vcg_operand_amax(x, (size_t)g.N * g.H * g.W * g.Cin, x_handle, WINO_V_SHIFT, st, &ax)) return -2;
-    V = (float*)ws;
-    p.amax_x = ax; p.vplanes = (unsigned short*)V;
-    hipLaunchKernelGGL(k_wino_in_tr, dim3(p.T / 32, p.Kc / 32), dim3(256), 0, st, p, (unsigned short*)v_keep);
-    VCG_LAUNCH_CHECK("vcg_conv_fwd(winograd input transform, + transposed)");
-    if (vcg_gemm_planes_batched(V, u, M, p.T, p.Kc, g.Cout, 16, ax, vcg_amax_stored(w_amax, WINO_U_SHIFT), st, keep_word)) return -2;
-  } else {
+  {
     VcgAmax ax;
     if (pre_bits) ax = vcg_amax_const(pre_bits, WINO_V_SHIFT);
     else if (vcg_operand_amax(x, (size_t)g.N * g.H * g.W * g.Cin, x_handle, WINO_V_SHIFT, st, &ax)) return -2;
diff --git a/vae-cyclegan-implementation_amd/csrc/gemm_split.hip b/vae-cyclegan-implementation_amd/csrc/gemm_split.hip
--- a/vae-cyclegan-implementation_amd/csrc/gemm_split.hip
+++ b/vae-cyclegan-implementation_amd/csrc/gemm_split.hip
@@ -159,6 +159,14 @@
 __device__ __forceinline__ void gd_barrier() {
   asm volatile("s_waitcnt lgkmcnt(0)\n\ts_barrier" ::: "memory");
 }
+typedef short gd_s16x4 __attribute__((ext_vector_type(4)));
+typedef short gd_s16x8 __attribute__((ext_vector_type(8)));
+__device__ __forceinline__ f16x8 gd_tr2(uint32_t a0, uint32_t a1) {
+  const gd_s16x4 lo = __builtin_amdgcn_ds_read_tr16_b64_v4i16((__attribute__((address_space(3))) gd_s16x4*)(uintptr_t)a0);
+  const gd_s16x4 hi = __builtin_amdgcn_ds_read_tr16_b64_v4i16((__attribute__((address_space(3))) gd_s16x4*)(uintptr_t)a1);
+  const gd_s16x8 v = {lo[0], lo[1], lo[2], lo[3], hi[0], hi[1], hi[2], hi[3]};
+  return __builtin_bit_cast(f16x8, v);
+}
 constexpr int GD_BM = 256, GD_BN = 128;
 constexpr int GD_A_BYTES = GD_BM * VCG_PBYTES, GD_B_BYTES = GD_BN * VCG_PBYTES;
 constexpr int GD_STAGE = GD_A_BYTES + GD_B_BYTES;
@@ -172,7 +180,8 @@
 #define GD_T() 0ull
 #define GD_ACC(slot, t0) do { } while (0)
 #endif
-__global__ __launch_bounds__(512, 1) void k_gemm_planes_dma(GemmSplitP p) {
+template <bool TN>
+__device__ __forceinline__ void gemm_planes_dma_body(const GemmSplitP& p) {
   __shared__ __attribute__((aligned(1024))) unsigned char smem[GD_STAGES * GD_STAGE];
   const int tid = threadIdx.x, lane = tid & 63, wid = tid >> 6;
   const int wm = wid >> 1, wn = wid & 1;
@@ -200,23 +209,45 @@
   const int KB = p.K / 32;
   const int drow = lane >> 3, dslot = lane & 7;
   uint32_t aoff[4], boff[2];
-#pragma unroll
-  for (int h = 0; h < 4; ++h) {
-    const int rl = (wid + 8 * h) * 8 + drow;
-    const int r = m0 + rl;
-    aoff[h] = r < p.rows ? (uint32_t)((size_t)r * KB * VCG_PBYTES + ((dslot ^ ((rl >> 1) & 7)) << 4)) : GS_OOB;
-  }
-#pragma unroll
-  for (int h = 0; h < 2; ++h) {
-    const int rl = (wid + 8 * h) * 8 + drow;
-    boff[h] = (uint32_t)((size_t)(n0 + rl) * KB * VCG_PBYTES + ((dslot ^ ((rl >> 1) & 7)) << 4));
+  uint32_t akstep = VCG_PBYTES, bkstep = VCG_PBYTES;
+  if constexpr (!TN) {
+#pragma unroll
+    for (int h = 0; h < 4; ++h) {
+      const int rl = (wid + 8 * h) * 8 + drow;
+      const int r = m0 + rl;
+      aoff[h] = r < p.rows ? (uint32_t)((size_t)r * KB * VCG_PBYTES + ((dslot ^ ((rl >> 1) & 7)) << 4)) : GS_OOB;
+    }
+#pragma unroll
+    for (int h = 0; h < 2; ++h) {
+      const int rl = (wid + 8 * h) * 8 + drow;
+      boff[h] = (uint32_t)((size_t)(n0 + rl) * KB * VCG_PBYTES + ((dslot ^ ((rl >> 1) & 7)) << 4));
+    }
+  } else {
+    const uint32_t arow = (uint32_t)(p.rows / 32) * VCG_PBYTES, brow = (uint32_t)(p.N / 32) * VCG_PBYTES;
+#pragma unroll
+    for (int h = 0; h < 4; ++h) {
+      const int tr = wid + 8 * h;
+      const int s = lane ^ (((tr & 3) | (((tr >> 3) & 1) << 2)) << 1);
+      aoff[h] = m0 + (s >> 3) * 32 < p.rows ? (uint32_t)tr * arow + (uint32_t)m0 * 4u + (uint32_t)s * 16u : GS_OOB;
+    }
+#pragma unroll
+    for (int h = 0; h < 2; ++h) {
+      const int tr = 2 * (wid + 8 * h) + (lane >> 5);
+      const int s = (lane & 31) ^ (((tr & 3) | (((tr >> 3) & 1) << 2)) << 1);
+      boff[h] = n0 + (s >> 3) * 32 < p.N ? (uint32_t)tr * brow + (uint32_t)n0 * 4u + (uint32_t)s * 16u : GS_OOB;
+    }
+    akstep = 32u * arow; bkstep = 32u * brow;
   }
   const uint32_t lds0 = (uint32_t)(uintptr_t)(__attribute__((address_space(3))) unsigned char*)smem;
   auto issue_one = [&](int stage, int kt, int q) {
     const uint32_t sbase = __builtin_amdgcn_readfirstlane(lds0 + (uint32_t)stage * GD_STAGE);
-    const uint32_t ko = (uint32_t)kt * VCG_PBYTES;
-    if (q < 4) gd_dma16(ra, __builtin_amdgcn_readfirstlane(sbase + (uint32_t)((wid + 8 * q) * 1024)), aoff[q] != GS_OOB ? aoff[q] + ko : GS_OOB);
-    else gd_dma16(rb, __builtin_amdgcn_readfirstlane(sbase + (uint32_t)(GD_A_BYTES + (wid + 8 * (q - 4)) * 1024)), boff[q - 4] + ko);
+    if (q < 4) {
+      gd_dma16(ra, __builtin_amdgcn_readfirstlane(sbase + (uint32_t)((wid + 8 * q) * 1024)), aoff[q] != GS_OOB ? aoff[q] + (uint32_t)kt * akstep : GS_OOB);
+    } else {
+      const uint32_t bo = boff[q - 4] + (uint32_t)kt * bkstep;
+      gd_dma16(rb, __builtin_amdgcn_readfirstlane(sbase + (uint32_t)(GD_A_BYTES + (wid + 8 * (q - 4)) * 1024)),
+               TN && boff[q - 4] == GS_OOB ? GS_OOB : bo);
+    }
   };
   auto issue = [&](int stage, int kt) {
 #pragma unroll
@@ -248,7 +279,24 @@
   unsigned long long gd_t = GD_T();
   (void)gd_t;
   f16x8 a16[VCG_NP][4], b16[VCG_NP][4];
+  const int tq = r16 >> 2, tp = lane & 3;
+  const uint32_t tfx = (uint32_t)((tq | ((kq & 1) << 2)) << 1);
+  const uint32_t ta = lds0 + (uint32_t)((8 * kq + tq) * 1024 + wm * 256 + 8 * tp);
+  const uint32_t tb = lds0 + (uint32_t)(GD_A_BYTES + (8 * kq + tq) * 512 + wn * 256 + 8 * tp);
   auto read16 = [&](int kt) {
+    if constexpr (TN) {
+      const uint32_t so = (uint32_t)(kt % GD_STAGES) * GD_STAGE;
+#pragma unroll
+      for (int pc = 0; pc < VCG_NP; ++pc) {
+#pragma unroll
+        for (int i = 0; i < 4; ++i) {
+          const uint32_t o = (((uint32_t)((i >> 1) * 8 + pc * 4 + (i & 1) * 2) ^ tfx) << 4) + so;
+          a16[pc][i] = gd_tr2(ta + o, ta + o + 4 * 1024);
+          b16[pc][i] = gd_tr2(tb + o, tb + o + 4 * 512);
+        }
+      }
+      return;
+    }
     const unsigned char* st = smem + (kt % GD_STAGES) * GD_STAGE;
 #pragma unroll
     for (int pc = 0; pc < VCG_NP; ++pc) {
@@ -326,6 +374,8 @@
   }
 #endif
 }
+__global__ __launch_bounds__(512, 1) void k_gemm_planes_dma(GemmSplitP p) { gemm_planes_dma_body<false>(p); }
+__global__ __launch_bounds__(512, 1) void k_gemm_planes_dma_tn(GemmSplitP p) { gemm_planes_dma_body<true>(p); }
 __global__ __launch_bounds__(256) void k_split_planes(const float* __restrict__ x, unsigned short* __restrict__ bp, size_t quads, int K, VcgAmax amax) {
   float s, inv;
   vcg_scale_of(vcg_amax_bits(amax), amax.shift, s, inv);
@@ -377,3 +427,25 @@
   VCG_LAUNCH_CHECK("vcg_gemm_planes_batched");
   return 0;
 }
+
+int vcg_gemm_planes_tn_batched(const void* APlanes, const void* BPlanes, float* C, int rows, int T, int N, int batches, const VcgAmax& amax_a,
+                               const VcgAmax& amax_b, hipStream_t st) {
+  VCG_CHECK_ARG(T > 0 && T % 32 == 0 && rows > 0 && rows % 32 == 0 && N > 0 && N % 32 == 0,
+                "vcg_gemm_planes_tn_batched: bad shape rows=%d T=%d N=%d", rows, T, N);
+  VCG_CHECK_ARG((unsigned long long)rows * T * 2 * VCG_NP < (1ull << 31) && (unsigned long long)N * T * 2 * VCG_NP < (1ull << 31),
+                "vcg_gemm_planes_tn_batched: operand extents must stay below 2 GiB per batch");
+  VCG_CHECK_ARG((unsigned long long)rows * T * VCG_NP * (unsigned long long)batches < (1ull << 32) &&
+                    (unsigned long long)N * T * VCG_NP * (unsigned long long)batches < (1ull << 32),
+                "vcg_gemm_planes_tn_batched: batch stride overflow");
+  GemmSplitP p;
+  p.a = (const float*)APlanes; p.bt = (const float*)BPlanes; p.c = C; p.rows = rows; p.K = T; p.N = N;
+  p.a_bytes = (uint32_t)((size_t)rows * T * 2 * VCG_NP); p.b_bytes = (uint32_t)((size_t)N * T * 2 * VCG_NP);
+  p.a_bstride = (uint32_t)((size_t)rows * T * VCG_NP); p.b_bstride = (uint32_t)((size_t)N * T * VCG_NP);
+  p.c_bstride = (size_t)rows * N;
+  p.amax_a = amax_a; p.amax_b = amax_b; p.amax_a_keep = nullptr;
+  dim3 grid((rows + GD_BM - 1) / GD_BM, (N + GD_BN - 1) / GD_BN, batches);
+  VcgProfScope prof("k_gemm_planes_dma", 2.0 * rows * (double)T * N * batches, st);
+  hipLaunchKernelGGL(k_gemm_planes_dma_tn, grid, dim3(512), 0, st, p);
+  VCG_LAUNCH_CHECK("vcg_gemm_planes_tn_batched");
+  return 0;
+}
```

Result: no change. 251.9 images/s, median of 6 (+1.8%).
